# hangg7/soar

Hardware: AMD Instinct MI355X
Metric: fwd+bwd frames/sec @100k Gaussians, 1080p; achieved HBM GB/s vs roofline (higher is better)
Workload: dtype f32

## Files before the change

### include/soar_hip.h

```cpp
#ifndef SOAR_HIP_H
#define SOAR_HIP_H

#include <stddef.h>
#include <stdint.h>

#ifdef __cplusplus
extern "C" {
#endif

#define SOAR_HIP_ABI_VERSION 8

typedef struct SoarRastParams {
    int32_t P;
    int32_t W, H;
    int32_t sh_degree;
    int32_t M;
    int32_t prefiltered;
    int32_t render_front;
    int32_t sort_descending;
    int32_t debug;
    int32_t cfg_surface;
    int32_t cfg_normalize_depth;
    int32_t cfg_perpix_depth;
    int32_t cfg_lrn_cam;
// ... 108 lines not shown
int soar_lbs_knn_weights_bytes(int32_t P, int32_t V, size_t *bytes);
int soar_lbs_knn_weights(const float *xyz, int32_t P, const float *verts, int32_t V,
                         const float *vert_weights, int32_t J, int32_t K,
                         float *weights_out, int32_t *knn_idx_out,
                         void *workspace, size_t workspace_bytes, void *stream);

int soar_lbs_knn_grid_bytes(int32_t V, size_t *bytes);
int soar_lbs_knn_query_bytes(int32_t P, size_t *bytes);
int soar_lbs_knn_build_grid(const float *verts, int32_t V, const float *vert_weights, int32_t J, void *grid_buffer,
                            void *stream);
int soar_lbs_knn_query(const void *grid_buffer, int32_t V, const float *vert_weights, int32_t J,
                       const float *xyz, int32_t P, int32_t K, float *weights_out, int32_t *knn_idx_out,
                       void *query_workspace, size_t query_workspace_bytes, void *stream);
int soar_lbs_knn_query_ordered(const void *grid_buffer, int32_t V, const float *vert_weights, int32_t J,
                               const float *xyz, int32_t P, int32_t K, uint32_t *order, int32_t resort,
                               float *weights_out, int32_t *knn_idx_out,
                               void *query_workspace, size_t query_workspace_bytes, void *stream);

int soar_lbs_knn_state_bytes(int32_t P, size_t *bytes);
int soar_lbs_knn_query_state(const void *grid_buffer, int32_t V, const float *vert_weights, int32_t J, const float *xyz, int32_t P,
                             uint32_t *order, int32_t resort, float *weights_out, void *state_buffer, void *query_workspace,
                             size_t query_workspace_bytes, void *stream);
int soar_lbs_knn_refresh(const void *grid_buffer, int32_t V, int32_t J, const float *xyz, int32_t P, const uint32_t *order,
                         void *state_buffer, float *weights_out, uint32_t *searched_counter_dev, void *stream);

int soar_lbs_warp_forward(const float *xyz, const float *rot, const float *weights, const float *joint_mats,
                          const float *offsets, const float *axis_perm, int32_t P, int32_t J,
                          float *xyz_out, float *rot_out, float *pt_mats_out, void *stream);

int soar_lbs_warp_backward(const float *xyz, const float *rot, const float *weights, const float *joint_mats,
                           const float *axis_perm, int32_t P, int32_t J,
                           const float *dL_dxyz_out, const float *dL_drot_out,
                           float *dL_dxyz, float *dL_drot, void *stream);

typedef struct SoarFrameHead {
    const SoarRastParams *prm;
    void *geom_buffer;
    int32_t *radii;
} SoarFrameHead;
int soar_frames_warp_preprocess(int32_t n, const SoarFrameHead *frames, const float *xyz, const float *rot, const float *weights,
                                const float *joint_mats, int32_t P, int32_t J, const float *colors, const float *opacities, const float *scales,
                                float *xyz_out, float *rot_out, void *stream);

int soar_rast_backward_rows(const SoarRastParams *prm, const float *means3D, const int32_t *radii, const float *shs, const float *scales,
                            const float *rotations, const float *cov3D_precomp, const void *geom_buffer, const void *workspace,
                            float *dL_dmeans2D, float *dL_dcolors, float *dL_dopacity, float *dL_dmeans3D, float *dL_dcov3D, float *dL_dsh,
                            float *dL_dscales, float *dL_drotations, float *dL_dviewmat, float *dL_dprojmat, float *dL_dcampos, float *dL_docc,
                            void *stream);

typedef struct SoarFrameTail {
    const SoarRastParams *prm;
    const float *means3D;
    const float *rotations;
    const int32_t *radii;
    const void *geom_buffer;
    const void *workspace;
    float *dL_dmeans2D;
} SoarFrameTail;
int soar_frames_geometry_warp_backward(int32_t n, const SoarFrameTail *frames, const float *xyz, const float *rot, const float *weights,
                                       const float *joint_mats, int32_t P, int32_t J, const float *scales, float *dL_dxyz, float *dL_drot,
                                       float *dL_dscales, float *dL_dcolors, float *dL_docc, void *stream);

int soar_lbs_warp_forward_batch(const float *xyz, const float *rot, const float *weights, const float *joint_mats, int32_t n,
                                int32_t P, int32_t J, float *xyz_out, float *rot_out, void *stream);
int soar_lbs_warp_backward_sum(const float *xyz, const float *rot, const float *weights, const float *joint_mats, int32_t n,
                               int32_t P, int32_t J, const float *dL_dxyz_out, const float *dL_drot_out, float *dL_dxyz,
                               float *dL_drot, int32_t n_extra, const float *const *extra_src, float *const *extra_dst,
                               const int32_t *extra_width, void *stream);

int soar_dist2_knn3(const float *points, int32_t N, float *out, void *stream);

#define SOAR_FRAME_LOSS_SCRATCH_FLOATS (4 * 2048)
int soar_frame_loss(int32_t W, int32_t H, const float *color, const float *normal, const float *depth,
                    const float *opac, const float *target_color, const float *target_mask,
                    const float *target_normal, float w_color, float w_mask, float w_normal, float w_depth,
                    float *loss_out, float *scratch, float *dL_dcolor, float *dL_dnormal, float *dL_ddepth,
                    float *dL_dopac, const void *image_buffer, const float *background, int32_t normalize_depth, void *stream);

int soar_frame_loss_pooled(int32_t W, int32_t H, const float *color, const float *normal, const float *depth,
                           const float *opac, const float *target_pool, int32_t n_sets, const int32_t *set_index_dev,
                           float w_color, float w_mask, float w_normal, float w_depth, float *loss_out, float *scratch,
                           float *dL_dcolor, float *dL_dnormal, float *dL_ddepth, float *dL_dopac, const void *image_buffer,
                           const float *background, int32_t normalize_depth, void *stream);

typedef struct SoarAvatarLossArgs {
    int32_t H, W;
    float cos_limit, cos_weight;
    const float *render, *gt_rgb;
    const float *mask_img, *gt_mask;
    const float *normal, *gt_normal;
    const float *occ;
    const uint8_t *sel, *sel_normal, *sel_occ;
    float *stats, *stats_occ;
    float *scratch;
    const float *counts;
    const float *up_l1, *up_l1m, *up_cos, *up_occ, *up_ssim;
    const float *g_ssim;
    float *g_render, *g_mask, *g_normal, *g_occ;
    int32_t normal_raw;
    int32_t occ_grad_summed;
    float *cos_scale_out;
    const float *background;
} SoarAvatarLossArgs;
int soar_avatar_loss_scratch_floats(size_t *count);
int soar_avatar_pixel_losses(const SoarAvatarLossArgs *args, int32_t mode, void *stream);

int soar_ssim_scratch_floats(int32_t C, int32_t H, int32_t W, size_t *count);
int soar_ssim(int32_t C, int32_t H, int32_t W, const float *img1, const float *img2, float *ssim_out, float *scratch,
              float *dssim_dimg1, void *stream);
int soar_ssim_rendered(int32_t C, int32_t H, int32_t W, const float *img1, const float *img2, float *ssim_out, float *scratch,
                       float *dssim_dimg1, const float *rendered, void *stream);

typedef struct SoarDensifyRow {
    const float *src;
    float *dst;
    int32_t width;
    int32_t mode;
} SoarDensifyRow;
int soar_densify_stats(int32_t P, const int32_t *radii, const float *grad2d, int32_t grad_stride, const float *scaling_grad,
                       const float *rotation, const float *opacity, float *accum, float *max_radii2D, void *stream);
int soar_densify_plan_bytes(int32_t P, size_t *bytes);
int soar_densify_plan(int32_t P, const float *accum, const float *scaling, const float *opacity, int32_t do_prune,
                      int32_t do_densify, float min_opacity, float prune_scale_max, float prune_area_min, float max_grad,
                      float dense_scale, void *plan, int64_t *counts_host, void *stream);
int soar_densify_flags(int32_t P, const void *plan, uint8_t *flags_out, void *stream);
int soar_densify_apply(int32_t P, int32_t N, const void *plan, int32_t n_rows, const SoarDensifyRow *rows, const float *scaling,
                       const float *rotation, const float *noise, int32_t surface, void *stream);

int soar_smplx_joint_mats(int32_t B, int32_t J, int32_t NB, const float *betas, int32_t betas_batch, const float *J_template,
                          const float *J_dirs, const int32_t *parents, const float *full_pose, const float *transl,
                          const float *right_mats, float *out, void *stream);

int soar_image_loss_scratch_floats(size_t *count);
int soar_masked_l1(int32_t C, int32_t H, int32_t W, const float *img, const float *gt, const uint8_t *mask, float *stats2,
                   float *scratch, void *stream);
int soar_masked_l1_backward(int32_t C, int32_t H, int32_t W, const float *img, const float *gt, const uint8_t *mask,
                            const float *stats2, const float *upstream_dev, float *dL_dimg, void *stream);
int soar_cos_loss(int32_t C, int32_t H, int32_t W, const float *output, const float *gt, const uint8_t *mask, float cos_thrsh,
                  float weight, float *stats2, float *scratch, void *stream);
int soar_cos_loss_backward(int32_t C, int32_t H, int32_t W, const float *output, const float *gt, const uint8_t *mask,
                           float cos_thrsh, float weight, const float *stats2, const float *upstream_dev, float *dL_doutput,
                           void *stream);

int soar_depth2normal(int32_t W, int32_t H, const float *depth, const uint8_t *mask, float prcp_x, float prcp_y,
                      float focal_k00, float focal_k11, float *normal_out, void *stream);
int soar_depth2normal_backward(int32_t W, int32_t H, const float *depth, const uint8_t *mask, float prcp_x, float prcp_y,
                               float focal_k00, float focal_k11, const float *dL_dnormal, float *dL_ddepth, void *stream);
int soar_normal2curv(int32_t W, int32_t H, const float *normal, const uint8_t *mask, float *curv_out, void *stream);
int soar_normal2curv_backward(int32_t W, int32_t H, const float *normal, const uint8_t *mask, const float *dL_dcurv,
                              float *dL_dnormal, void *stream);

int soar_view_finish(int32_t W, int32_t H, const float *normal, const float *depth, const float *opac,
                     const float *prcppoint_dev, float focal_k00, float focal_k11, float *normal_out, float *curv_out,
                     float *pred_normal_out, void *stream);
int soar_view_finish_backward(int32_t W, int32_t H, const float *normal, const float *depth, const float *opac,
                              const float *prcppoint_dev, float focal_k00, float focal_k11, const float *dL_dnormal_out,
                              const float *dL_dcurv, const float *dL_dpred_normal, const float *dL_ddepth_direct,
                              float *dL_dnormal_and_depth, void *stream);

typedef struct SoarPoseArgs {
    int32_t P, J;
    int32_t scale_width;
    int32_t warp;
    const float *xyz, *rot;
    const float *weights;
    const float *joint_mats;
    const float *offsets;
    const float *axis_perm;
    const float *colors;
    const float *scale_src;
    const float *occ;
    float *occ3;
    float *posed;
    float *grad_scratch;
    float *dL_dxyz, *dL_drot, *dL_dcolors, *dL_dscale;
    float *dL_docc;
} SoarPoseArgs;
typedef struct SoarViewArgs {
    SoarRastParams rast;
    float focal_k00, focal_k11;
    int32_t back;
    int32_t pad_;
    int64_t capacity;
    void *buffer;
    size_t buffer_bytes;
    float *out;
    int32_t *radii;
    uint32_t *status_pinned;
    const float *g_render, *g_normal, *g_depth, *g_pred_normal, *g_mask, *g_occ, *g_curv;
    float *dL_dmeans2D;
} SoarViewArgs;
int soar_view_buffer_bytes(int32_t P, int32_t W, int32_t H, int64_t capacity, int32_t back, size_t *bytes);
int soar_views_grad_scratch_floats(int32_t P, int32_t n_views, size_t *floats);
int soar_views_forward(const SoarPoseArgs *pose, int32_t n_views, const SoarViewArgs *views, void *stream);
int soar_views_backward(const SoarPoseArgs *pose, int32_t n_views, const SoarViewArgs *views, void *stream);
int soar_step_views_forward(int32_t n_poses, const SoarPoseArgs *poses, const int32_t *views_per_pose, const SoarViewArgs *views, void *stream);
int soar_step_views_backward(int32_t n_poses, const SoarPoseArgs *poses, const int32_t *views_per_pose, const SoarViewArgs *views, void *stream);
typedef struct SoarCameraSpec {
    double fovx, fovy, znear, zfar;
    double cx, cy, img_w, img_h;
    int32_t has_cxcy, pad_;
} SoarCameraSpec;
int soar_cameras_from_c2w(int32_t n, const float *c2w_dev, const float *c2w_host, const SoarCameraSpec *specs, float *out_dev, void *stream);
int soar_rast_forward_render_status(const SoarRastParams *prm, const int32_t *radii, void *geom_buffer, void *binning_buffer,
                                    void *image_buffer, int64_t num_rendered, float *out_color, float *out_normal, float *out_depth,
                                    float *out_opac, const float *occ_values, float *out_occ, uint32_t *status_pinned, void *stream);
int soar_lbs_warp_backward_views(const float *xyz, const float *rot, const float *weights, const float *joint_mats, const float *axis_perm,
                                 int32_t n, int32_t P, int32_t J, const float *dL_dxyz_out, const float *dL_drot_out, float *dL_dxyz,
                                 float *dL_drot, int32_t n_extra, const float *const *extra_src, float *const *extra_dst,
                                 const int32_t *extra_width, void *stream);

int soar_prof_enable(int on);
int soar_prof_reset(void);
int soar_prof_stage_count(void);
const char *soar_prof_stage_name(int stage);
int soar_prof_read(int stage, double *total_ms, int64_t *launches);
int soar_sum_frames(int32_t n_frames, int64_t count, const float *in_dev, float *out_dev, void *stream);
int soar_gather_step_inputs(int32_t n_frames, int32_t num_frames_seq, int32_t floats_per_frame, int32_t n_sets,
                            const int32_t *frame_ids_dev, const float *table_dev, float *mats_out_dev,
                            int32_t *set_index_out_dev, void *stream);
int soar_gather_step_inputs_ids(int32_t n_frames, int32_t num_frames_seq, int32_t floats_per_frame, int32_t n_sets,
                                const int32_t *frame_ids_host, const float *table_dev, float *mats_out_dev,
                                int32_t *set_index_out_dev, void *stream);

typedef struct SoarAdamRow {
    float *param;
    const float *grad;
    float *exp_avg;
    float *exp_avg_sq;
    int64_t count;
    float lr;
    int32_t pad_;
} SoarAdamRow;
int soar_adam_step(int32_t n_rows, const SoarAdamRow *rows_host, double beta1, double beta2, double eps, void *state_dev, void *stream);
int soar_adam_step_at(int32_t n_rows, const SoarAdamRow *rows, double beta1, double beta2, double eps, int64_t step, void *stream);
int soar_adam_step_rows(int32_t n_rows, const SoarAdamRow *rows, double beta1, double beta2, double eps, void *state_dev, int32_t advance,
                        void *stream);
int soar_adam_step_rows_wide(int32_t n_rows, const SoarAdamRow *rows, double beta1, double beta2, double eps, void *state_dev,
                             int32_t advance, void *stream);

int soar_prof_timestamp(unsigned long long *ring_dev, int64_t capacity, int64_t tag, void *stream);

int soar_selftest_affine_scan(const float *m64_dev, const float *b64_dev, float *out192_dev, void *stream);

int soar_selftest_exp(const float *x_dev, int32_t n, float *out_dev, float *expf_dev, void *stream);

int soar_tsdf_integrate(int32_t n_views, int32_t H, int32_t W, const float *depth, const float *opac, const float *viewmatrix,
                        const float *projmatrix, const float *prcppoint, float origin_x, float origin_y, float origin_z, float voxel,
                        int32_t X, int32_t Y, int32_t Z, float trunc, float znear, float min_opacity, float *sum, float *weight,
                        void *stream);
int soar_mc_workspace_bytes(int32_t X, int32_t Y, int32_t Z, size_t *bytes);
int soar_mc_count(int32_t X, int32_t Y, int32_t Z, const float *values, const uint8_t *valid, float level, void *workspace,
                  size_t workspace_bytes, int64_t *counts_host, void *stream);
int soar_mc_emit(int32_t X, int32_t Y, int32_t Z, const float *values, const uint8_t *valid, float level, const void *workspace,
                 size_t workspace_bytes, float *verts, int32_t *faces, void *stream);
int soar_mesh_filter_bytes(int32_t V, int32_t F, size_t *bytes);
int soar_mesh_filter_components(int32_t V, int32_t F, const float *verts, const int32_t *faces, int32_t min_faces, float min_diag_frac,
                                void *workspace, size_t workspace_bytes, float *verts_out, int32_t *faces_out, int64_t *counts_host,
                                void *stream);

#define SOAR_FIELD_LEVELS 16
#define SOAR_FIELD_HIDDEN 64
#define SOAR_FIELD_HEAD_FLOATS(in, out) (SOAR_FIELD_HIDDEN * (in) + SOAR_FIELD_HIDDEN + (out) * SOAR_FIELD_HIDDEN + (out))
typedef struct SoarFieldHead {
    const float *w1, *b1, *w2, *b2;
} SoarFieldHead;

typedef struct SoarFieldArgs {
    int32_t N;
    int32_t log2_T;
    int32_t normalized;
    int32_t pad_;
    float res[SOAR_FIELD_LEVELS];
    const float *xyz;
    const float *aabb;
    const float *table, *qtable;
    const float *z;
    SoarFieldHead head[5];
    float *enc, *qenc;
    float *out[5];
    const float *g_out[5];
    float *d_table, *d_qtable;
    float *d_head[5];
    float *d_xyz, *d_z;
} SoarFieldArgs;

int soar_field_workspace_bytes(int32_t N, size_t *bytes);
int soar_field_forward(const SoarFieldArgs *args, void *stream);
int soar_field_backward(const SoarFieldArgs *args, void *workspace, size_t workspace_bytes, void *stream);

#define SOAR_ENVMAP_ENC 9
#define SOAR_ENVMAP_HIDDEN 16
#define SOAR_ENVMAP_WEIGHTS (SOAR_ENVMAP_HIDDEN * SOAR_ENVMAP_ENC + SOAR_ENVMAP_HIDDEN * SOAR_ENVMAP_HIDDEN + 3 * SOAR_ENVMAP_HIDDEN)
typedef struct SoarEnvmapArgs {
    int32_t B, H, W;
    int32_t n_comp;
    int32_t color_rows;
    int32_t pad_;
    int64_t render_stride, mask_stride;
    int64_t g_comp_stride[4];
    const float *dirs;
    const float *w1, *w2, *w3;
    const float *color;
    const float *render, *mask;
    float *bg;
    float *comp;
// ... 138 lines not shown
```

### soar_amd/csrc/api.hip

```cpp
#include "soar_common.h"

#include <mutex>

#include <dlfcn.h>

#include <cstdarg>
#include <cstdio>
#include <cstring>

namespace soar {

static thread_local char g_error[1024] = "";

void set_error(const char *fmt, ...)
{
    va_list ap;
    va_start(ap, fmt);
    vsnprintf(g_error, sizeof(g_error), fmt, ap);
    va_end(ap);
}

int check_hip(hipError_t e, const char *what, const char *file, int line)
{
    if (e == hipSuccess) return 0;
    set_error("HIP error %d (%s) in %s at %s:%d", (int)e, hipGetErrorString(e), what, file, line);
    return 1;
}

int post_launch(const char *what, hipStream_t stream, int debug)
{
    hipError_t e = hipGetLastError();
    if (e == hipSuccess && (debug & 1)) e = hipStreamSynchronize(stream);
    if (e == hipSuccess) return 0;
    set_error("stage '%s' failed: HIP error %d (%s)", what, (int)e, hipGetErrorString(e));
    return 1;
}

BatchCtx &batch_ctx()
{
    static thread_local BatchCtx ctx;
    return ctx;
}

namespace {
constexpr int ZERO_RANGES = 5;
struct ZeroArgs { uint32_t *ptr[ZERO_RANGES]; size_t words[ZERO_RANGES]; size_t first_block[ZERO_RANGES + 1]; };
constexpr int ZERO_UNROLL = 8;
constexpr size_t ZERO_BLOCK_WORDS = 256 * 4 * ZERO_UNROLL;
__global__ void __launch_bounds__(256) zero_ranges_kernel(Batch<ZeroArgs> b)
{
    const ZeroArgs &z = b.v[blockIdx.y];
    if (blockIdx.x >= z.first_block[ZERO_RANGES]) return;
    int r = 0;
    while (r < ZERO_RANGES - 1 && blockIdx.x >= z.first_block[r + 1]) r++;
    const size_t b0 = ((size_t)blockIdx.x - z.first_block[r]) * ZERO_BLOCK_WORDS;
    uint32_t *p = z.ptr[r];
    const size_t n = z.words[r];
    if (b0 + ZERO_BLOCK_WORDS <= n && (reinterpret_cast<uintptr_t>(p) & 15) == 0) {
#pragma unroll
        for (int u = 0; u < ZERO_UNROLL; u++)
            *reinterpret_cast<uint4 *>(p + b0 + (size_t)u * 1024 + threadIdx.x * 4) = make_uint4(0u, 0u, 0u, 0u);
    } else {
        for (size_t w = b0 + threadIdx.x; w < n && w < b0 + ZERO_BLOCK_WORDS; w += 256) p[w] = 0u;
    }
}
}

int launch_zero_ranges(const ZeroRange *ranges, int count, hipStream_t stream)
{
    ZeroArgs z;
    size_t blocks = 0;
    if (count > ZERO_RANGES) { set_error("launch_zero_ranges: at most %d ranges", ZERO_RANGES); return 1; }
    for (int r = 0; r < ZERO_RANGES; r++) {
        z.first_block[r] = blocks;
        z.ptr[r] = r < count ? static_cast<uint32_t *>(ranges[r].ptr) : nullptr;
        z.words[r] = r < count ? ranges[r].bytes / 4 : 0;
        blocks += (z.words[r] + ZERO_BLOCK_WORDS - 1) / ZERO_BLOCK_WORDS;
    }
    z.first_block[ZERO_RANGES] = blocks;
    if (blocks == 0) return 0;
    SOAR_LAUNCH_BATCHED(zero_ranges_kernel, dim3((unsigned)blocks), dim3(256), 0, stream, z);
    return post_launch("zero_ranges", stream, 0);
}

namespace {
struct ProfSlot { hipEvent_t a, b; int stage; bool open; };
constexpr int PROF_SLOTS = 16384;
std::mutex g_prof_mutex;
bool g_prof_on = false;
ProfSlot g_slots[PROF_SLOTS];
int g_slot_used = 0;
bool g_slots_init = false;
double g_stage_ms[ST_COUNT];
long long g_stage_n[ST_COUNT];
const char *g_stage_names[ST_COUNT] = {"preprocess", "scan", "tile_lists", "depth_order", "tile_ranges", "render_forward",
                                       "render_backward", "geometry_backward", "lbs_knn_weights", "lbs_warp_forward",
                                       "lbs_warp_backward", "dist2_knn3", "frame_loss", "postops", "block_masks", "optimizer"};
void prof_drain()
{
    for (int i = 0; i < g_slot_used; i++) {
        float ms = 0.f;
        if (hipEventSynchronize(g_slots[i].b) == hipSuccess && hipEventElapsedTime(&ms, g_slots[i].a, g_slots[i].b) == hipSuccess) {
            g_stage_ms[g_slots[i].stage] += ms;
            g_stage_n[g_slots[i].stage] += 1;
        }
    }
    g_slot_used = 0;
}
}

namespace {
struct Roctx {
    int (*push)(const char *) = nullptr;
    int (*pop)() = nullptr;
    Roctx()
    {
        const char *on = getenv("SOAR_ROCTX");
        if (!on || on[0] == '0') return;
        void *h = dlopen("librocprofiler-sdk-roctx.so", RTLD_NOW | RTLD_GLOBAL);
        if (!h) h = dlopen("libroctx64.so", RTLD_NOW | RTLD_GLOBAL);
        if (!h) return;
        push = reinterpret_cast<int (*)(const char *)>(dlsym(h, "roctxRangePushA"));
        pop = reinterpret_cast<int (*)()>(dlsym(h, "roctxRangePop"));
        if (!push || !pop) push = nullptr;
    }
};
const Roctx &roctx()
{
    static const Roctx r;
    return r;
}
}

StageTimer::StageTimer(int stage, hipStream_t s) : slot(-1), stream(s)
{
    marked = roctx().push != nullptr;
    if (marked) (void)roctx().push(g_stage_names[stage]);
    if (!g_prof_on) return;
    if (batch_ctx().n && batch_ctx().f != batch_ctx().n - 1) return;
    {
        std::lock_guard<std::mutex> lock(g_prof_mutex);
        if (!g_slots_init) {
            for (int i = 0; i < PROF_SLOTS; i++) { (void)hipEventCreate(&g_slots[i].a); (void)hipEventCreate(&g_slots[i].b); }
            g_slots_init = true;
        }
        if (g_slot_used == PROF_SLOTS) return;
        slot = g_slot_used++;
        g_slots[slot].stage = stage;
    }
    (void)hipEventRecord(g_slots[slot].a, stream);
}
StageTimer::~StageTimer()
{
    if (slot >= 0) (void)hipEventRecord(g_slots[slot].b, stream);
    if (marked) (void)roctx().pop();
}

template <typename T>
static void take(char *&p, T *&ptr, size_t count)
{
    p = reinterpret_cast<char *>(align_up(reinterpret_cast<size_t>(p)));
    ptr = reinterpret_cast<T *>(p);
// ... 446 lines not shown
                                     binning_buffer, image_buffer, num_rendered, dL_dout_color, dL_dout_normal, dL_dout_depth,
                                     dL_dout_opac, nullptr, dL_dmeans2D, dL_dcolors, dL_dopacity, dL_dmeans3D, dL_dcov3D, dL_dsh,
                                     dL_dscales, dL_drotations, dL_dviewmat, dL_dprojmat, dL_dcampos, workspace, workspace_bytes,
                                     stream_);
}

int soar_rast_backward_rows(const SoarRastParams *prm, const float *means3D, const int32_t *radii, const float *shs, const float *scales,
                            const float *rotations, const float *cov3D_precomp, const void *geom_buffer, const void *workspace,
                            float *dL_dmeans2D, float *dL_dcolors, float *dL_dopacity, float *dL_dmeans3D, float *dL_dcov3D, float *dL_dsh,
                            float *dL_dscales, float *dL_drotations, float *dL_dviewmat, float *dL_dprojmat, float *dL_dcampos, float *dL_docc,
                            void *stream_)
{
    hipStream_t stream = static_cast<hipStream_t>(stream_);
    if (check_params(prm)) return 1;
    if (prm->P == 0) return 0;
    if (check_aligned(geom_buffer, "geom_buffer") || check_aligned(workspace, "workspace")) return 1;
    if (!means3D || !radii || !dL_dmeans2D || !dL_dcolors || !dL_dopacity || !dL_dmeans3D || !dL_dcov3D || !dL_dscales || !dL_drotations ||
        !dL_dviewmat || !dL_dprojmat || !dL_dcampos) {
        set_error("soar_rast_backward_rows: a required pointer is NULL");
        return 1;
    }
    GeomBuf g;
    carve_geom(const_cast<void *>(geom_buffer), prm->P, prm->M, &g);
    return launch_geometry_backward(*prm, means3D, radii, shs, scales, rotations, cov3D_precomp, g, static_cast<const float *>(workspace),
                                    dL_dmeans2D, dL_dcolors, dL_dopacity, dL_dmeans3D, dL_dcov3D, dL_dsh, dL_dscales, dL_drotations,
                                    dL_dviewmat, dL_dprojmat, dL_dcampos, true, stream, dL_docc);
}

}

static int backward_impl(const SoarRastParams *prm, const float *means3D, const int32_t *radii, const float *shs,
                              const float *colors_precomp, const float *scales, const float *rotations,
                              const float *cov3D_precomp, const void *geom_buffer, const void *binning_buffer,
                              const void *image_buffer, int64_t num_rendered, const float *dL_dout_color,
                              const float *dL_dout_normal, const float *dL_dout_depth, const float *dL_dout_opac,
                              const float *grad_scale_dev, float *dL_dmeans2D, float *dL_dcolors, float *dL_dopacity,
                              float *dL_dmeans3D, float *dL_dcov3D, float *dL_dsh, float *dL_dscales, float *dL_drotations,
                              float *dL_dviewmat, float *dL_dprojmat, float *dL_dcampos, void *workspace,
                              size_t workspace_bytes, const float *dL_dout_occ, float *dL_docc, const float *normal_scale_dev, int occ_planes,
                              void *stream_)
{
    hipStream_t stream = static_cast<hipStream_t>(stream_);
    if (check_params(prm)) return 1;
    if (!dL_dviewmat || !dL_dprojmat || !dL_dcampos) { set_error("camera gradient pointers must not be NULL"); return 1; }
    if ((dL_dout_occ == nullptr) != (dL_docc == nullptr)) { set_error("soar_rast_backward_occ: dL_dout_occ and dL_docc go together"); return 1; }
    if (dL_dout_occ && (prm->render_front != 0 || prm->sort_descending != 0)) {
        set_error("soar_rast_backward_occ: the fused occlusion chain belongs to a main pass (render_front = 0, ascending)");
        return 1;
    }
    if (prm->P == 0) {
        SOAR_HIP_OK(hipMemsetAsync(dL_dviewmat, 0, 16 * sizeof(float), stream));
        SOAR_HIP_OK(hipMemsetAsync(dL_dprojmat, 0, 16 * sizeof(float), stream));
        SOAR_HIP_OK(hipMemsetAsync(dL_dcampos, 0, 3 * sizeof(float), stream));
        return 0;
    }
    if (check_aligned(geom_buffer, "geom_buffer") || check_aligned(image_buffer, "image_buffer") ||
        check_aligned(workspace, "workspace"))
        return 1;
    if (num_rendered > 0 && check_aligned(binning_buffer, "binning_buffer")) return 1;
    size_t need = 0;
    soar_rast_backward_workspace_bytes(prm->P, &need);
    if (workspace_bytes < need - ALIGN) { set_error("workspace too small: %zu < %zu", workspace_bytes, need); return 1; }
    if (!means3D || !radii || !dL_dout_color || !dL_dout_normal || !dL_dout_depth || !dL_dout_opac || !dL_dmeans2D ||
        !dL_dcolors || !dL_dopacity || !dL_dmeans3D || !dL_dcov3D || !dL_dscales || !dL_drotations) {
        set_error("soar_rast_backward: a required pointer is NULL");
        return 1;
    }
    if (prm->M > 0 && shs && !dL_dsh) { set_error("dL_dsh is NULL but SHs are in use"); return 1; }
    (void)colors_precomp;

    GeomBuf g;
    ImageBuf img;
    BinBuf b;
    carve_geom(const_cast<void *>(geom_buffer), prm->P, prm->M, &g);
    carve_image(const_cast<void *>(image_buffer), prm->W, prm->H, &img);
    carve_binning(const_cast<void *>(binning_buffer), num_rendered, &b);
    float *acc = static_cast<float *>(workspace);
    const bool wide = (prm->debug & 2) != 0;
    double *acc64 = wide ? reinterpret_cast<double *>(static_cast<char *>(workspace) + align_up(sizeof(float) * ACC_STRIDE * (size_t)prm->P))
                         : nullptr;
    {
        const ZeroRange zr[4] = {{wide ? (void *)acc64 : (void *)acc, (wide ? sizeof(double) : sizeof(float)) * ACC_STRIDE * (size_t)prm->P},
                                 {dL_dviewmat, 16 * sizeof(float)}, {dL_dprojmat, 16 * sizeof(float)}, {dL_dcampos, 3 * sizeof(float)}};
        if (launch_zero_ranges(zr, 4, stream)) return 1;
    }
    if (num_rendered > 0 || wide) {
        if (launch_render_backward(*prm, g, b, img, dL_dout_color, dL_dout_normal, dL_dout_depth, dL_dout_opac, grad_scale_dev, acc,
                                   acc64, num_rendered > 0, dL_dout_occ, dL_docc, normal_scale_dev, occ_planes, stream))
            return 1;
    }
    if ((prm->debug & 8) != 0) return 0;
    if (launch_geometry_backward(*prm, means3D, radii, shs, scales, rotations, cov3D_precomp, g, acc, dL_dmeans2D, dL_dcolors,
                                 dL_dopacity, dL_dmeans3D, dL_dcov3D, dL_dsh, dL_dscales, dL_drotations, dL_dviewmat,
                                 dL_dprojmat, dL_dcampos, false, stream, dL_docc))
        return 1;
    return 0;
}


extern "C" {

int soar_rast_backward_scaled(const SoarRastParams *prm, const float *means3D, const int32_t *radii, const float *shs,
                              const float *colors_precomp, const float *scales, const float *rotations,
                              const float *cov3D_precomp, const void *geom_buffer, const void *binning_buffer,
                              const void *image_buffer, int64_t num_rendered, const float *dL_dout_color,
                              const float *dL_dout_normal, const float *dL_dout_depth, const float *dL_dout_opac,
                              const float *grad_scale_dev, float *dL_dmeans2D, float *dL_dcolors, float *dL_dopacity,
                              float *dL_dmeans3D, float *dL_dcov3D, float *dL_dsh, float *dL_dscales, float *dL_drotations,
                              float *dL_dviewmat, float *dL_dprojmat, float *dL_dcampos, void *workspace,
                              size_t workspace_bytes, void *stream_)
{
    return backward_impl(prm, means3D, radii, shs, colors_precomp, scales, rotations, cov3D_precomp, geom_buffer, binning_buffer, image_buffer,
                         num_rendered, dL_dout_color, dL_dout_normal, dL_dout_depth, dL_dout_opac, grad_scale_dev, dL_dmeans2D, dL_dcolors,
                         dL_dopacity, dL_dmeans3D, dL_dcov3D, dL_dsh, dL_dscales, dL_drotations, dL_dviewmat, dL_dprojmat, dL_dcampos, workspace,
                         workspace_bytes, nullptr, nullptr, nullptr, 3, stream_);
}

int soar_rast_backward_occ(const SoarRastParams *prm, const float *means3D, const int32_t *radii, const float *shs,
                           const float *colors_precomp, const float *scales, const float *rotations,
                           const float *cov3D_precomp, const void *geom_buffer, const void *binning_buffer,
                           const void *image_buffer, int64_t num_rendered, const float *dL_dout_color,
                           const float *dL_dout_normal, const float *dL_dout_depth, const float *dL_dout_opac,
                           const float *dL_dout_occ, const float *normal_scale_dev, int32_t occ_planes, float *dL_dmeans2D, float *dL_dcolors,
                           float *dL_dopacity,
                           float *dL_dmeans3D, float *dL_dcov3D, float *dL_dsh, float *dL_dscales, float *dL_drotations,
                           float *dL_dviewmat, float *dL_dprojmat, float *dL_dcampos, float *dL_docc, void *workspace,
                           size_t workspace_bytes, void *stream_)
{
    if (!dL_dout_occ || !dL_docc) { set_error("soar_rast_backward_occ: dL_dout_occ / dL_docc must not be NULL"); return 1; }
    if (occ_planes != 1 && occ_planes != 3) { set_error("soar_rast_backward_occ: occ_planes is 3 or 1, got %d", occ_planes); return 1; }
    return backward_impl(prm, means3D, radii, shs, colors_precomp, scales, rotations, cov3D_precomp, geom_buffer, binning_buffer, image_buffer,
                         num_rendered, dL_dout_color, dL_dout_normal, dL_dout_depth, dL_dout_opac, nullptr, dL_dmeans2D, dL_dcolors,
                         dL_dopacity, dL_dmeans3D, dL_dcov3D, dL_dsh, dL_dscales, dL_drotations, dL_dviewmat, dL_dprojmat, dL_dcampos, workspace,
                         workspace_bytes, dL_dout_occ, dL_docc, normal_scale_dev, occ_planes, stream_);
}

int soar_rast_mark_visible(int32_t P, const float *means3D, const float *viewmatrix, const float *projmatrix,
                           uint8_t *present, void *stream_)
{
    (void)means3D; (void)viewmatrix; (void)projmatrix;
    hipStream_t stream = static_cast<hipStream_t>(stream_);
    if (P < 0) { set_error("P < 0"); return 1; }
    if (P == 0) return 0;
    if (!present) { set_error("present is NULL"); return 1; }
    SOAR_HIP_OK(hipMemsetAsync(present, 0, (size_t)P, stream));
    return 0;
}

}

namespace soar {
namespace {
__global__ void export_records_kernel(int P, const GaussRec *rec, float *means2D, float *depths, float *conic_opacity,
                                      float *normal, float *depth_plane, float *rgb)
{
    const int i = blockIdx.x * blockDim.x + threadIdx.x;
    if (i >= P) return;
    const GaussRec r = rec[i];
    if (means2D) { means2D[2 * i] = r.q0.x; means2D[2 * i + 1] = r.q0.y; }
    if (depths) depths[i] = r.q1.z;
    if (conic_opacity) {
        conic_opacity[4 * i] = r.q0.z; conic_opacity[4 * i + 1] = r.q0.w; conic_opacity[4 * i + 2] = r.q1.x;
        conic_opacity[4 * i + 3] = r.q1.y;
    }
    if (normal) { normal[3 * i] = r.q3.x; normal[3 * i + 1] = r.q3.y; normal[3 * i + 2] = r.q3.z; }
    if (depth_plane) { depth_plane[2 * i] = r.q1.w; depth_plane[2 * i + 1] = r.q2.x; }
    if (rgb) { rgb[3 * i] = r.q2.y; rgb[3 * i + 1] = r.q2.z; rgb[3 * i + 2] = r.q2.w; }
// ... 105 lines not shown
```

### soar_amd/csrc/frame_loss.hip

```cpp
#include "soar_common.h"

#include <type_traits>

namespace soar {

namespace {

struct LossArgs {
    int n;
    const float *color, *normal, *depth, *opac;
    const float *t_color, *t_mask, *t_normal;
    float wc, wm, wn, wd;
    float *dcolor, *dnormal, *ddepth, *dopac;
    float *sums;
    const int *set_index;
    int n_sets;
    const float *bg;
    int normalize_depth;
    const uint32_t *n_contrib;
    const uint32_t *bg_tiles;
    int W, gx;
};

__device__ __forceinline__ float sign_of(float v) { return v > 0.f ? 1.f : (v < 0.f ? -1.f : 0.f); }

__device__ __forceinline__ float wave_sum(float v)
{
#pragma unroll
    for (int off = 32; off > 0; off >>= 1) v += __shfl_xor(v, off);
    return v;
}

template <int V> struct Vec;
template <> struct Vec<4> { typedef float4 type; };
template <> struct Vec<1> { typedef float type; };
__device__ __forceinline__ float4 ld(const float4 *p, int i) { return p[i]; }
__device__ __forceinline__ float4 ld(const float *p, int i) { return make_float4(p[i], 0.f, 0.f, 0.f); }
__device__ __forceinline__ void st(float4 *p, int i, float4 v) { p[i] = v; }
__device__ __forceinline__ void st(float *p, int i, float4 v) { p[i] = v.x; }
__device__ __forceinline__ bool any_contrib(const uint4 *p, int i) { const uint4 v = p[i]; return (v.x | v.y | v.z | v.w) != 0u; }
__device__ __forceinline__ bool any_contrib(const uint32_t *p, int i) { return p[i] != 0u; }

template <int V>
__global__ void __launch_bounds__(256) frame_loss_kernel(Batch<LossArgs> batch)
{
    LossArgs a = batch.v[blockIdx.y];
    typedef typename Vec<V>::type T;
    const int nv = a.n / V;
    if (a.set_index) {
        const float *set = a.t_color + (size_t)((unsigned)*a.set_index % (unsigned)a.n_sets) * 7u * (size_t)a.n;
        a.t_color = set; a.t_mask = set + 3 * (size_t)a.n; a.t_normal = set + 4 * (size_t)a.n;
    }
    float s_c = 0.f, s_m = 0.f, s_n = 0.f, s_d = 0.f;
    const float gc = a.wc / (3.f * a.n), gm = a.wm / a.n, gn = a.wn / (3.f * a.n), gd = a.wd / a.n;
    const float4 pad = V == 4 ? make_float4(1.f, 1.f, 1.f, 1.f) : make_float4(1.f, 0.f, 0.f, 0.f);
    typedef typename std::conditional<V == 4, uint4, uint32_t>::type U;
    const float Tc = (float)(1 - 0.000001);
    const bool known = a.n_contrib && a.bg;
    float bgc[3] = {0.f, 0.f, 0.f};
    if (known) { bgc[0] = 0.f + Tc * a.bg[0]; bgc[1] = 0.f + Tc * a.bg[1]; bgc[2] = 0.f + Tc * a.bg[2]; }
    const float bg_depth = a.normalize_depth ? 0.f / (1.f - Tc) : 0.f + Tc * 10.f, bg_opac = 1.f - Tc;
    for (int i = blockIdx.x * 256 + threadIdx.x; i < nv; i += gridDim.x * 256) {
        bool wr = true;
        if (a.n_contrib) {
            bool empty_tile = false;
            if (a.bg_tiles) {
                const int p = i * V, y = p / a.W, x = p - y * a.W;
                empty_tile = a.bg_tiles[(y >> 4) * a.gx + (x >> 4)] != 0u;
            }
            wr = !empty_tile && any_contrib(reinterpret_cast<const U *>(a.n_contrib), i);
        }
        const bool rd = wr || !known;
        float4 nsum = make_float4(0.f, 0.f, 0.f, 0.f);
#pragma unroll
        for (int ch = 0; ch < 3; ch++) {
            const float4 c = rd ? ld(reinterpret_cast<const T *>(a.color + (size_t)ch * a.n), i) : make_float4(bgc[ch], bgc[ch], bgc[ch], bgc[ch]);
            const float4 t = ld(reinterpret_cast<const T *>(a.t_color + (size_t)ch * a.n), i);
            const float4 d = make_float4(c.x - t.x, c.y - t.y, c.z - t.z, c.w - t.w);
            s_c += (fabsf(d.x) + fabsf(d.y)) + (fabsf(d.z) + fabsf(d.w));
            if (wr) st(reinterpret_cast<T *>(a.dcolor + (size_t)ch * a.n), i,
                       make_float4(gc * sign_of(d.x), gc * sign_of(d.y), gc * sign_of(d.z), gc * sign_of(d.w)));
            const float4 nr = rd ? ld(reinterpret_cast<const T *>(a.normal + (size_t)ch * a.n), i) : make_float4(0.f, 0.f, 0.f, 0.f);
            const float4 nt = rd ? ld(reinterpret_cast<const T *>(a.t_normal + (size_t)ch * a.n), i) : make_float4(0.f, 0.f, 0.f, 0.f);
            nsum.x += nr.x * nt.x; nsum.y += nr.y * nt.y; nsum.z += nr.z * nt.z; nsum.w += nr.w * nt.w;
            if (wr) st(reinterpret_cast<T *>(a.dnormal + (size_t)ch * a.n), i, make_float4(gn * nt.x, gn * nt.y, gn * nt.z, gn * nt.w));
        }
        s_n += (nsum.x + nsum.y) + (nsum.z + nsum.w);
        const float4 o = rd ? ld(reinterpret_cast<const T *>(a.opac), i) : make_float4(bg_opac, bg_opac, bg_opac, bg_opac);
        const float4 m = ld(reinterpret_cast<const T *>(a.t_mask), i);
        const float4 e = make_float4(o.x - m.x, o.y - m.y, o.z - m.z, o.w - m.w);
        s_m += (fabsf(e.x) + fabsf(e.y)) + (fabsf(e.z) + fabsf(e.w));
        if (wr) st(reinterpret_cast<T *>(a.dopac), i, make_float4(gm * sign_of(e.x), gm * sign_of(e.y), gm * sign_of(e.z), gm * sign_of(e.w)));
        const float4 dp = rd ? ld(reinterpret_cast<const T *>(a.depth), i) : make_float4(bg_depth, bg_depth, bg_depth, bg_depth);
        s_d += (dp.x + dp.y) + (dp.z + dp.w);
        if (wr) st(reinterpret_cast<T *>(a.ddepth), i, make_float4(gd * pad.x, gd * pad.y, gd * pad.z, gd * pad.w));
    }
    __shared__ float part[4][4];
    s_c = wave_sum(s_c); s_m = wave_sum(s_m); s_n = wave_sum(s_n); s_d = wave_sum(s_d);
    const int wave = threadIdx.x >> 6, lane = threadIdx.x & 63;
    if (lane == 0) { part[wave][0] = s_c; part[wave][1] = s_m; part[wave][2] = s_n; part[wave][3] = s_d; }
    __syncthreads();
    if (threadIdx.x < 4)
        a.sums[4 * blockIdx.x + threadIdx.x] = (part[0][threadIdx.x] + part[1][threadIdx.x]) + (part[2][threadIdx.x] + part[3][threadIdx.x]);
}

struct LossFinishArgs {
    const float *sums;
    int blocks, n;
    float wc, wm, wn, wd;
    float *loss;
};
__global__ void __launch_bounds__(256) frame_loss_finish_kernel(Batch<LossFinishArgs> batch)
{
    const LossFinishArgs &fa = batch.v[blockIdx.y];
    const float *sums = fa.sums;
    const int blocks = fa.blocks, n = fa.n;
    const float wc = fa.wc, wm = fa.wm, wn = fa.wn, wd = fa.wd;
    float *loss = fa.loss;
    __shared__ float4 red[256];
    float4 acc = make_float4(0.f, 0.f, 0.f, 0.f);
    for (int b = threadIdx.x; b < blocks; b += 256) {
        const float4 v = reinterpret_cast<const float4 *>(sums)[b];
        acc.x += v.x; acc.y += v.y; acc.z += v.z; acc.w += v.w;
    }
    red[threadIdx.x] = acc;
    __syncthreads();
    for (int off = 128; off > 0; off >>= 1) {
        if ((int)threadIdx.x < off) {
            const float4 o = red[threadIdx.x + off];
            float4 m = red[threadIdx.x];
            m.x += o.x; m.y += o.y; m.z += o.z; m.w += o.w;
            red[threadIdx.x] = m;
        }
        __syncthreads();
    }
    if (threadIdx.x == 0) {
        const float4 S = red[0];
        *loss = (wc * S.x / (3.f * n) + wm * S.y / n) + (wn * S.z / (3.f * n) + wd * S.w / n);
    }
}

}

}

using namespace soar;

static int frame_loss_launch(int32_t W, int32_t H, const float *color, const float *normal, const float *depth, const float *opac,
                             const float *target_color, const float *target_mask, const float *target_normal,
                             const int32_t *set_index_dev, int32_t n_sets, float w_color, float w_mask, float w_normal,
                             float w_depth, float *loss_out, float *sums4, float *dL_dcolor, float *dL_dnormal, float *dL_ddepth,
                             float *dL_dopac, const void *image_buffer, const float *background, int32_t normalize_depth, hipStream_t stream);

extern "C" int soar_frame_loss(int32_t W, int32_t H, const float *color, const float *normal, const float *depth,
                               const float *opac, const float *target_color, const float *target_mask,
                               const float *target_normal, float w_color, float w_mask, float w_normal, float w_depth,
                               float *loss_out, float *sums4, float *dL_dcolor, float *dL_dnormal, float *dL_ddepth,
                               float *dL_dopac, const void *image_buffer, const float *background, int32_t normalize_depth,
                               void *stream_)
{
    return frame_loss_launch(W, H, color, normal, depth, opac, target_color, target_mask, target_normal, nullptr, 1, w_color,
                             w_mask, w_normal, w_depth, loss_out, sums4, dL_dcolor, dL_dnormal, dL_ddepth, dL_dopac, image_buffer,
                             background, normalize_depth, static_cast<hipStream_t>(stream_));
}

extern "C" int soar_frame_loss_pooled(int32_t W, int32_t H, const float *color, const float *normal, const float *depth,
                                      const float *opac, const float *target_pool, int32_t n_sets,
                                      const int32_t *set_index_dev, float w_color, float w_mask, float w_normal, float w_depth,
                                      float *loss_out, float *sums4, float *dL_dcolor, float *dL_dnormal, float *dL_ddepth,
                                      float *dL_dopac, const void *image_buffer, const float *background,
                                      int32_t normalize_depth, void *stream_)
{
    if (n_sets <= 0 || !set_index_dev) { set_error("soar_frame_loss_pooled: need n_sets > 0 and a device index"); return 1; }
    return frame_loss_launch(W, H, color, normal, depth, opac, target_pool, target_pool, target_pool, set_index_dev, n_sets,
                             w_color, w_mask, w_normal, w_depth, loss_out, sums4, dL_dcolor, dL_dnormal, dL_ddepth, dL_dopac,
                             image_buffer, background, normalize_depth, static_cast<hipStream_t>(stream_));
}

static int frame_loss_launch(int32_t W, int32_t H, const float *color, const float *normal, const float *depth, const float *opac,
                             const float *target_color, const float *target_mask, const float *target_normal,
                             const int32_t *set_index_dev, int32_t n_sets, float w_color, float w_mask, float w_normal,
                             float w_depth, float *loss_out, float *sums4, float *dL_dcolor, float *dL_dnormal, float *dL_ddepth,
                             float *dL_dopac, const void *image_buffer, const float *background, int32_t normalize_depth, hipStream_t stream)
{
    if (W <= 0 || H <= 0) { set_error("soar_frame_loss: bad image size %dx%d", W, H); return 1; }
    if (!color || !normal || !depth || !opac || !target_color || !target_mask || !target_normal || !loss_out || !sums4 ||
        !dL_dcolor || !dL_dnormal || !dL_ddepth || !dL_dopac) {
        set_error("soar_frame_loss: NULL pointer");
        return 1;
    }
    LossArgs a;
    a.n = W * H;
    a.color = color; a.normal = normal; a.depth = depth; a.opac = opac;
    a.t_color = target_color; a.t_mask = target_mask; a.t_normal = target_normal;
    a.wc = w_color; a.wm = w_mask; a.wn = w_normal; a.wd = w_depth;
    a.dcolor = dL_dcolor; a.dnormal = dL_dnormal; a.ddepth = dL_ddepth; a.dopac = dL_dopac;
    a.sums = sums4;
    a.set_index = set_index_dev; a.n_sets = n_sets;
    a.n_contrib = nullptr; a.bg_tiles = nullptr; a.W = W; a.gx = (W + TILE - 1) / TILE;
    a.bg = image_buffer ? background : nullptr; a.normalize_depth = normalize_depth;
    if (image_buffer) {
        ImageBuf img;
        carve_image(const_cast<void *>(image_buffer), W, H, &img);
        a.n_contrib = img.n_contrib;
        if (W % 4 == 0) a.bg_tiles = img.bg_tiles;
    }
    StageTimer timer(ST_FRAME_LOSS, stream);
    const bool vec4 = (a.n & 3) == 0 && (((uintptr_t)a.n_contrib | (uintptr_t)color | (uintptr_t)normal | (uintptr_t)depth | (uintptr_t)opac | (uintptr_t)target_color |
                                          (uintptr_t)target_mask | (uintptr_t)target_normal | (uintptr_t)dL_dcolor | (uintptr_t)dL_dnormal |
                                          (uintptr_t)dL_ddepth | (uintptr_t)dL_dopac) & 15) == 0;
    const int blocks = min(SOAR_FRAME_LOSS_SCRATCH_FLOATS / 4, max(1, (a.n / (vec4 ? 4 : 1) + 255) / 256));
    if (vec4) SOAR_LAUNCH_BATCHED(frame_loss_kernel<4>, dim3(blocks), dim3(256), 0, stream, a);
    else SOAR_LAUNCH_BATCHED(frame_loss_kernel<1>, dim3(blocks), dim3(256), 0, stream, a);
    const soar::LossFinishArgs fa = {sums4, blocks, a.n, w_color, w_mask, w_normal, w_depth, loss_out};
    SOAR_LAUNCH_BATCHED(frame_loss_finish_kernel, dim3(1), dim3(256), 0, stream, fa);
    SOAR_LAUNCH_OK("frame_loss", stream, 0);
    return 0;
}


namespace soar {
namespace {
template <int VEC>
__global__ void __launch_bounds__(256) sum_frames_kernel(int n_frames, size_t count, const float *__restrict__ in, float *__restrict__ out)
{
    const size_t i = ((size_t)blockIdx.x * 256 + threadIdx.x) * VEC;
    if (i >= count) return;
    if (VEC == 4) {
        float4 acc = *reinterpret_cast<const float4 *>(in + i);
        for (int f = 1; f < n_frames; f++) {
            const float4 v = *reinterpret_cast<const float4 *>(in + (size_t)f * count + i);
            acc.x += v.x; acc.y += v.y; acc.z += v.z; acc.w += v.w;
        }
        *reinterpret_cast<float4 *>(out + i) = acc;
    } else {
        float acc = in[i];
        for (int f = 1; f < n_frames; f++) acc += in[(size_t)f * count + i];
        out[i] = acc;
    }
}
__global__ void gather_step_inputs_kernel(int n_frames, int num_frames_seq, int floats_per_frame, int n_sets,
                                          const int32_t *__restrict__ frame_ids, const float *__restrict__ table,
                                          float *__restrict__ mats_out, int32_t *__restrict__ set_out)
{
    const int f = blockIdx.x;
    int id = frame_ids[f] % num_frames_seq;
    if (id < 0) id += num_frames_seq;
    for (int k = threadIdx.x; k < floats_per_frame; k += blockDim.x) mats_out[(size_t)f * floats_per_frame + k] = table[(size_t)id * floats_per_frame + k];
    if (threadIdx.x == 0 && set_out) set_out[f] = n_sets > 0 ? id % n_sets : 0;
}
struct StepFrameIds { int32_t id[MAX_BATCH]; };
__global__ void gather_step_inputs_ids_kernel(int n_frames, int num_frames_seq, int floats_per_frame, int n_sets, StepFrameIds ids,
                                              const float *__restrict__ table, float *__restrict__ mats_out, int32_t *__restrict__ set_out)
{
    const int f = blockIdx.x;
    int id = ids.id[f] % num_frames_seq;
    if (id < 0) id += num_frames_seq;
    for (int k = threadIdx.x; k < floats_per_frame; k += blockDim.x) mats_out[(size_t)f * floats_per_frame + k] = table[(size_t)id * floats_per_frame + k];
    if (threadIdx.x == 0 && set_out) set_out[f] = n_sets > 0 ? id % n_sets : 0;
}
}
}

extern "C" int soar_sum_frames(int32_t n_frames, int64_t count, const float *in_dev, float *out_dev, void *stream_)
{
    using namespace soar;
    hipStream_t stream = static_cast<hipStream_t>(stream_);
    if (n_frames <= 0 || count < 0 || !in_dev || !out_dev) { set_error("soar_sum_frames: bad arguments"); return 1; }
    if (count == 0) return 0;
    const bool vec = ((((uintptr_t)in_dev | (uintptr_t)out_dev) & 15) == 0) && ((count & 3) == 0);
    if (vec) hipLaunchKernelGGL(sum_frames_kernel<4>, dim3((unsigned)((count / 4 + 255) / 256)), dim3(256), 0, stream, n_frames, (size_t)count, in_dev, out_dev);
    else hipLaunchKernelGGL(sum_frames_kernel<1>, dim3((unsigned)((count + 255) / 256)), dim3(256), 0, stream, n_frames, (size_t)count, in_dev, out_dev);
    SOAR_LAUNCH_OK("sum_frames", stream, 0);
    return 0;
}

extern "C" int soar_gather_step_inputs(int32_t n_frames, int32_t num_frames_seq, int32_t floats_per_frame, int32_t n_sets,
                                       const int32_t *frame_ids_dev, const float *table_dev, float *mats_out_dev,
                                       int32_t *set_index_out_dev, void *stream_)
{
    using namespace soar;
    hipStream_t stream = static_cast<hipStream_t>(stream_);
    if (n_frames <= 0 || num_frames_seq <= 0 || floats_per_frame <= 0 || !frame_ids_dev || !table_dev || !mats_out_dev) {
        set_error("soar_gather_step_inputs: bad arguments");
        return 1;
    }
    hipLaunchKernelGGL(gather_step_inputs_kernel, dim3(n_frames), dim3(256), 0, stream, n_frames, num_frames_seq, floats_per_frame, n_sets,
                       frame_ids_dev, table_dev, mats_out_dev, set_index_out_dev);
    SOAR_LAUNCH_OK("gather_step_inputs", stream, 0);
    return 0;
}

extern "C" int soar_gather_step_inputs_ids(int32_t n_frames, int32_t num_frames_seq, int32_t floats_per_frame, int32_t n_sets,
                                           const int32_t *frame_ids_host, const float *table_dev, float *mats_out_dev,
                                           int32_t *set_index_out_dev, void *stream_)
{
    using namespace soar;
    hipStream_t stream = static_cast<hipStream_t>(stream_);
    if (n_frames <= 0 || n_frames > MAX_BATCH || num_frames_seq <= 0 || floats_per_frame <= 0 || !frame_ids_host || !table_dev || !mats_out_dev) {
        set_error("soar_gather_step_inputs_ids: bad arguments (at most %d frames per step)", MAX_BATCH);
        return 1;
    }
    StepFrameIds ids = {};
    for (int f = 0; f < n_frames; f++) ids.id[f] = frame_ids_host[f];
    hipLaunchKernelGGL(gather_step_inputs_ids_kernel, dim3(n_frames), dim3(256), 0, stream, n_frames, num_frames_seq, floats_per_frame, n_sets, ids,
                       table_dev, mats_out_dev, set_index_out_dev);
    SOAR_LAUNCH_OK("gather_step_inputs", stream, 0);
    return 0;
}
```

### soar_amd/csrc/lbs_knn.hip

```cpp
#include "soar_common.h"

#include <cstdio>
#include <cstdlib>
#include <cstring>
#include <rocprim/device/device_radix_sort.hpp>

namespace soar {

namespace {

constexpr int KNN_THREADS = 128;
constexpr int KNN_MAXK = 32;
constexpr int GRID_MAX = 64;
constexpr int GRID_RES = 28;
constexpr int KNN_K = 30;
constexpr int KNN_JMAX = 56;
constexpr int GRID_CELLS = GRID_MAX * GRID_MAX * GRID_MAX;

struct GridMeta {
    float minx, miny, minz, h, inv_h;
    int nx, ny, nz;
};

__global__ void __launch_bounds__(256) grid_meta_kernel(const float *__restrict__ verts, int V, GridMeta *meta)
// ... 336 lines not shown
    for (int k = 0; k < K; k++) {
        v[k] = fminf(best[k], other[(K - 1 - k) * stride]);
        tau = fmaxf(tau, v[k]);
    }
    need = K;
#pragma unroll
    for (int k = 0; k < K; k++) need -= (v[k] < tau) ? 1 : 0;
    return tau;
}

constexpr uint32_t KNN_ORDER_STAMP = 0x534F4152u;
__global__ void __launch_bounds__(WAVE)
item_cost_kernel(const uint32_t *__restrict__ q_keys, int P, const GridMeta *__restrict__ meta, const uint2 *__restrict__ cell_range,
                 uint32_t *__restrict__ cost)
{
    const int lane = threadIdx.x, chunk = blockIdx.x, q = chunk * WAVE + lane;
    const bool valid = q < P;
    const uint32_t key = valid ? q_keys[q] : 0xFFFFFFFFu;
    const GridMeta m = *meta;
    uint32_t item[KNN_SLOTS];
#pragma unroll
    for (int k = 0; k < KNN_SLOTS; k++) item[k] = 0u;
    unsigned long long remaining = __ballot(valid);
    for (int seg = 0; remaining != 0ull; seg++) {
        const uint32_t c = (uint32_t)__builtin_amdgcn_readlane((int)key, (int)__builtin_ctzll(remaining));
        const unsigned long long mine = __ballot(valid && key == c);
        remaining &= ~mine;
        const int cx = (int)(c % GRID_MAX), cy = (int)((c / GRID_MAX) % GRID_MAX), cz = (int)(c / (GRID_MAX * GRID_MAX));
        uint32_t n = 0;
        if (lane < 27) {
            const int gx = cx + lane % 3 - 1, gy = cy + (lane / 3) % 3 - 1, gz = cz + lane / 9 - 1;
            if (gx >= 0 && gx < m.nx && gy >= 0 && gy < m.ny && gz >= 0 && gz < m.nz) {
                const uint2 rg = cell_range[(gz * GRID_MAX + gy) * GRID_MAX + gx];
                n = rg.y - rg.x;
            }
        }
#pragma unroll
        for (int off = 16; off > 0; off >>= 1) n += (uint32_t)__shfl_xor((int)n, off);
        n = (uint32_t)__builtin_amdgcn_readfirstlane((int)n);
        if (n < 2u * KNN_K) {
            uint32_t n5 = 0;
            for (int t = lane; t < 125; t += WAVE) {
                const int gx = cx + t % 5 - 2, gy = cy + (t / 5) % 5 - 2, gz = cz + t / 25 - 2;
                if (gx >= 0 && gx < m.nx && gy >= 0 && gy < m.ny && gz >= 0 && gz < m.nz) {
                    const uint2 rg = cell_range[(gz * GRID_MAX + gy) * GRID_MAX + gx];
                    n5 += rg.y - rg.x;
                }
            }
#pragma unroll
            for (int off = 32; off > 0; off >>= 1) n5 += (uint32_t)__shfl_xor((int)n5, off);
            n += (uint32_t)__builtin_amdgcn_readfirstlane((int)n5);
        }
        const uint32_t us100 = 8u * n + 70u * (uint32_t)__builtin_popcountll(mine) + 1200u;
#pragma unroll
        for (int k = 0; k < KNN_SLOTS; k++) item[k] += (seg % KNN_SLOTS) == k ? us100 : 0u;
    }
    if (lane < KNN_SLOTS) cost[chunk * KNN_SLOTS + lane] = lane == 0 ? item[0] : lane == 1 ? item[1] : lane == 2 ? item[2] : item[3];
}
__global__ void __launch_bounds__(1024) item_order_kernel(const uint32_t *__restrict__ cost, int n_items, uint32_t *__restrict__ order)
{
    __shared__ uint32_t count[33], cursor[33];
    const int tid = threadIdx.x;
    if (tid < 33) count[tid] = 0u;
    __syncthreads();
    auto class_of = [&](uint32_t c) -> int { return c == 0u ? 32 : 31 - (int)min(31u, c / 400u); };
    for (int i = tid; i < n_items; i += 1024) atomicAdd(&count[class_of(cost[i])], 1u);
    __syncthreads();
    if (tid == 0) {
        uint32_t acc = 0;
        for (int k = 0; k < 33; k++) { cursor[k] = acc; acc += count[k]; }
    }
    __syncthreads();
    for (int i = tid; i < n_items; i += 1024) order[atomicAdd(&cursor[class_of(cost[i])], 1u)] = (uint32_t)i;
    if (tid == 0) order[n_items] = KNN_ORDER_STAMP ^ (uint32_t)n_items;
}

template <bool WITH_IDX>
__global__ void __launch_bounds__(KNN_WAVES *WAVE) __attribute__((amdgpu_waves_per_eu(5, 8)))
knn_cell_kernel(const float *__restrict__ xyz, int P, int V, const GridMeta *__restrict__ meta,
                const uint2 *__restrict__ cell_range, const float4 *__restrict__ sorted_verts,
                const uint32_t *__restrict__ q_keys, const uint32_t *__restrict__ q_ids,
                const float *__restrict__ rows_padded, int J, float *__restrict__ weights_out,
                int32_t *__restrict__ knn_idx_out, const uint32_t *__restrict__ item_order,
                KnnStatePtrs state)
{
    constexpr int K = KNN_K;
    __shared__ float4 cand[KNN_CAND];
    __shared__ uint32_t row_start[KNN_ROWS], row_prefix[KNN_ROWS + 1];
    __shared__ int info[4];
    __shared__ float merge[2][K][WAVE];
    __shared__ float tau_s[WAVE];
    __shared__ int need_s[WAVE];
    __shared__ uint32_t list_pos[KNN_WAVES][WAVE];
    __shared__ float list_w[KNN_WAVES][WAVE];

    const int wave = threadIdx.x >> 6, lane = threadIdx.x & 63;
    const uint32_t n_items = gridDim.x;
    const bool ordered = item_order && item_order[n_items] == (KNN_ORDER_STAMP ^ n_items);
    const uint32_t n_chunks = n_items / KNN_SLOTS;
    const uint32_t item = ordered ? min(item_order[blockIdx.x], n_items - 1u) : (blockIdx.x % n_chunks) * KNN_SLOTS + blockIdx.x / n_chunks;
    const int chunk = (int)(item / KNN_SLOTS), slot = (int)(item % KNN_SLOTS);
    const int q = chunk * WAVE + lane;
    const bool valid = q < P;
    const uint32_t key = valid ? q_keys[q] : 0xFFFFFFFFu;
    unsigned long long remaining = __ballot(valid);
    if (remaining == 0ull) return;

    const int p = valid ? (int)q_ids[q] : 0;
    const float x = xyz[3 * p], y = xyz[3 * p + 1], z = xyz[3 * p + 2];
    const GridMeta m = *meta;
    const float qx = x - m.minx, qy = y - m.miny, qz = z - m.minz;

    for (int seg = 0; remaining != 0ull; seg++) {
        const int head = (int)__builtin_ctzll(remaining);
        const uint32_t c = (uint32_t)__builtin_amdgcn_readlane((int)key, head);
        const bool active = valid && key == c;
        remaining &= ~__ballot(active);
        if ((seg % KNN_SLOTS) != slot) continue;
        const int cx = (int)(c % GRID_MAX), cy = (int)((c / GRID_MAX) % GRID_MAX), cz = (int)(c / (GRID_MAX * GRID_MAX));

        int r = 1, n_rows = 0, N = 0;
        for (;; r++) {
            __syncthreads();
            if (wave == 0) box_rows(cell_range, m, cx, cy, cz, r, V, row_start, row_prefix, info, lane);
            __syncthreads();
            N = info[0];
            n_rows = info[1];
            float best[K];
#pragma unroll
            for (int k = 0; k < K; k++) best[k] = 3.0e38f;
            for (int base = 0; base < N; base += KNN_CAND) {
                const int n = min(KNN_CAND, N - base);
                if (base > 0) __syncthreads();
                stage_candidates(sorted_verts, row_start, row_prefix, n_rows, base, n, cand);
                __syncthreads();
#pragma unroll 2
                for (int i = wave; i < n; i += KNN_WAVES) chain_insert<K>(best, dist2_exact(x, y, z, cand[i]));
            }
            if (wave >= 2) {
#pragma unroll
                for (int k = 0; k < K; k++) merge[wave - 2][k][lane] = best[k];
            }
            __syncthreads();
            if (wave < 2) merge_sorted<K>(best, &merge[wave][0][lane], WAVE);
            __syncthreads();
            if (wave == 1) {
#pragma unroll
                for (int k = 0; k < K; k++) merge[0][k][lane] = best[k];
            }
            __syncthreads();
            if (wave == 0) {
                int need;
                const float tau = merge_sorted_kth<K>(best, &merge[0][0][lane], WAVE, need);
                tau_s[lane] = tau;
                need_s[lane] = need;
                float bound = 3.0e38f;
                bool open = false;
                if (cx - r > 0) { open = true; bound = fminf(bound, qx - (cx - r) * m.h); }
                if (cx + r < m.nx - 1) { open = true; bound = fminf(bound, (cx + r + 1) * m.h - qx); }
                if (cy - r > 0) { open = true; bound = fminf(bound, qy - (cy - r) * m.h); }
                if (cy + r < m.ny - 1) { open = true; bound = fminf(bound, (cy + r + 1) * m.h - qy); }
                if (cz - r > 0) { open = true; bound = fminf(bound, qz - (cz - r) * m.h); }
                if (cz + r < m.nz - 1) { open = true; bound = fminf(bound, (cz + r + 1) * m.h - qz); }
                bound = fmaxf(bound, 0.f) * 0.9999f;
                const bool certified = !open || r > KNN_RMAX || tau <= bound * bound;
                const bool final_box = __ballot(active && !certified) == 0ull;
                if (lane == 0) info[2] = final_box ? 1 : 0;
            }
            __syncthreads();
            if (info[2]) break;
        }
        const float tau = tau_s[lane];
        const int need = need_s[lane];

        const bool single = N <= KNN_CAND;
        float norm_lane = 0.f;
        int cnt_lane = 0;
        int need_left = need;
        uint32_t *lpos = list_pos[wave];
        float *lw = list_w[wave];
// ... 117 lines not shown
constexpr int KNN_FSLOTS = 4;
struct KnnSlots { uint2 list[KNN_FSLOTS][KNN_KEEP]; int p[KNN_FSLOTS]; };
__device__ __forceinline__ void slots_fill_pair(KnnSlots &sl, int slot_lo, int p, uint32_t mask, uint32_t pos, float d2, int lane)
{
    const int slot = slot_lo + (lane >> 5), l5 = lane & (KNN_KEEP - 1);
    if (p >= 0 && ((mask >> l5) & 1u)) {
        const int at = __builtin_popcount(mask & ((1u << l5) - 1u));
        sl.list[slot][at] = make_uint2(pos * (uint32_t)(KNN_JMAX * sizeof(float)), __float_as_uint(1.0f / fminf(fmaxf(sqrtf(d2), 0.0001f), 1.0f)));
    }
    if (l5 == 0) sl.p[slot] = p;
}
template <int UNROLL>
__device__ __forceinline__ void slots_blend(KnnSlots &sl, int lane, const float *__restrict__ rows_padded, int J,
                                            float *__restrict__ weights_out)
{
    static_assert(KNN_K % 2 == 0 && KNN_JMAX % 4 == 0 && KNN_JMAX / 4 <= 16 && KNN_FSLOTS * 16 == WAVE && KNN_KEEP * 2 == WAVE &&
                  KNN_JMAX * sizeof(float) <= KNN_KEEP * sizeof(uint2) && KNN_JMAX <= WAVE, "slot layout");
    __builtin_amdgcn_fence(__ATOMIC_RELEASE, "wavefront");
    __builtin_amdgcn_wave_barrier();
    __builtin_amdgcn_fence(__ATOMIC_ACQUIRE, "wavefront");
    const int g = lane >> 4, t = lane & 15;
    const int p = sl.p[g];
    if (p >= 0) {
        const uint32_t t16 = (uint32_t)min(t, KNN_JMAX / 4 - 1) * 16u;
        const char *rows_bytes = reinterpret_cast<const char *>(rows_padded);
        const uint4 *mine = reinterpret_cast<const uint4 *>(sl.list[g]);
        float4 acc = make_float4(0.f, 0.f, 0.f, 0.f);
        float norm = 0.f;
#pragma unroll UNROLL
        for (int k2 = 0; k2 < KNN_K / 2; k2++) {
            const uint4 e = mine[k2];
            const float4 r0 = *reinterpret_cast<const float4 *>(rows_bytes + (e.x + t16));
            const float4 r1 = *reinterpret_cast<const float4 *>(rows_bytes + (e.z + t16));
            const float w0 = __uint_as_float(e.y), w1 = __uint_as_float(e.w);
            acc.x = __builtin_fmaf(w0, r0.x, acc.x); acc.y = __builtin_fmaf(w0, r0.y, acc.y);
            acc.z = __builtin_fmaf(w0, r0.z, acc.z); acc.w = __builtin_fmaf(w0, r0.w, acc.w);
            norm += w0;
            acc.x = __builtin_fmaf(w1, r1.x, acc.x); acc.y = __builtin_fmaf(w1, r1.y, acc.y);
            acc.z = __builtin_fmaf(w1, r1.z, acc.z); acc.w = __builtin_fmaf(w1, r1.w, acc.w);
            norm += w1;
        }
        float4 *mine_out = reinterpret_cast<float4 *>(sl.list[g]);
        if (t < KNN_JMAX / 4) mine_out[t] = make_float4(acc.x / norm, acc.y / norm, acc.z / norm, acc.w / norm);
    }
    __builtin_amdgcn_fence(__ATOMIC_RELEASE, "wavefront");
    __builtin_amdgcn_wave_barrier();
    __builtin_amdgcn_fence(__ATOMIC_ACQUIRE, "wavefront");
#pragma unroll
    for (int r = 0; r < KNN_FSLOTS; r++) {
        const int pr = sl.p[r];
        if (pr >= 0 && lane < J) weights_out[(size_t)pr * J + lane] = reinterpret_cast<const float *>(sl.list[r])[lane];
    }
    __builtin_amdgcn_fence(__ATOMIC_RELEASE, "wavefront");
    __builtin_amdgcn_wave_barrier();
}

__device__ __forceinline__ uint32_t rank_32_halves(float d2, int lane, float &h30)
{
    const int l5 = lane & (KNN_KEEP - 1), base = lane & KNN_KEEP;
    int rank = 0;
#pragma unroll
    for (int j = 0; j < KNN_KEEP; j++) {
        const float dj = __shfl(d2, base + j);
        rank += (dj < d2 || (dj == d2 && j < l5)) ? 1 : 0;
    }
    const bool in = rank < KNN_K;
    float d_in = in ? d2 : 0.f, d_out = in ? 3.0e38f : d2;
#pragma unroll
    for (int off = KNN_KEEP / 2; off > 0; off >>= 1) {
        d_in = fmaxf(d_in, __shfl_xor(d_in, off));
        d_out = fminf(d_out, __shfl_xor(d_out, off));
    }
    h30 = half_gap(d_in, d_out);
    const unsigned long long b = __ballot(in);
    return (uint32_t)(base ? (b >> 32) : b);
}

#ifndef SOAR_KNN_CERT_PAIRS
#define SOAR_KNN_CERT_PAIRS 2
#endif
constexpr int KNN_CERT_PAIRS = SOAR_KNN_CERT_PAIRS;
__global__ void __launch_bounds__(KNN_WAVES *WAVE)
knn_certify_kernel(const float *__restrict__ xyz, int P, const float4 *__restrict__ sorted_verts, const uint32_t *__restrict__ order,
                   KnnStatePtrs st)
{
    const int wave = threadIdx.x >> 6, lane = threadIdx.x & 63, l5 = lane & (KNN_KEEP - 1);
    const int q_base = ((int)blockIdx.x * KNN_WAVES + wave) * (2 * KNN_CERT_PAIRS) + (lane >> 5);
    if (q_base - (lane >> 5) >= P) return;
    int qs[KNN_CERT_PAIRS];
    float4 ra[KNN_CERT_PAIRS], rb[KNN_CERT_PAIRS], vv[KNN_CERT_PAIRS];
    float xs[KNN_CERT_PAIRS], ys[KNN_CERT_PAIRS], zs[KNN_CERT_PAIRS];
#pragma unroll
    for (int i = 0; i < KNN_CERT_PAIRS; i++) {
        qs[i] = q_base + 2 * i;
        const int qc = min(qs[i], P - 1);
        const int p = order ? (int)order[qc] : qc;
        const uint32_t pos = st.nbr[(size_t)qc * KNN_STATE_STRIDE + l5];
        ra[i] = st.ref30[qc]; rb[i] = st.ref32[qc];
        xs[i] = xyz[3 * p]; ys[i] = xyz[3 * p + 1]; zs[i] = xyz[3 * p + 2];
        vv[i] = sorted_verts[pos];
    }
#pragma unroll
    for (int i = 0; i < KNN_CERT_PAIRS; i++) {
        const int q = qs[i];
        const bool valid = q < P;
        const float x = xs[i], y = ys[i], z = zs[i];
        const float d2 = dist2_exact(x, y, z, vv[i]);
        const float ax = x - ra[i].x, ay = y - ra[i].y, az = z - ra[i].z, bx = x - rb[i].x, by = y - rb[i].y, bz = z - rb[i].z;
        const float moved_a = __builtin_amdgcn_sqrtf((ax * ax + ay * ay) + az * az) * 1.0001f + 1.0e-12f;
        const float moved_b = __builtin_amdgcn_sqrtf((bx * bx + by * by) + bz * bz) * 1.0001f + 1.0e-12f;
        const bool ok_a = ra[i].w > 0.f && moved_a < ra[i].w, ok_b = rb[i].w > 0.f && moved_b < rb[i].w;
        const bool tier3 = valid && !ok_a && !ok_b, tier2 = valid && !ok_a && ok_b;
        if (__ballot(tier3)) {
            float far = d2;
#pragma unroll
            for (int off = KNN_KEEP / 2; off > 0; off >>= 1) far = fmaxf(far, __shfl_xor(far, off));
            if (tier3 && l5 == 0) {
                const uint32_t list = knn_work_list_of((uint32_t)q);
                uint32_t *item = knn_work_item(st.work, P, list, atomicAdd(st.work + list * KNN_WORK_LINE, 1u));
                item[0] = (uint32_t)q;
                item[1] = __float_as_uint(far);
            }
        }
        if (__ballot(tier2)) {
            float h30;
            const uint32_t mask = rank_32_halves(d2, lane, h30);
            if (tier2 && l5 == 0) { st.ref30[q] = make_float4(x, y, z, h30); st.in30[q] = mask; }
        }
        if (valid) st.d2[(size_t)q * KNN_STATE_STRIDE + l5] = tier3 ? -1.f : d2;
    }
}

#ifndef SOAR_KNN_SEARCH_BLOCKS
#define SOAR_KNN_SEARCH_BLOCKS 768
#endif
#ifndef SOAR_KNN_BS_WPE
#define SOAR_KNN_BS_WPE 4
#endif
__global__ void __launch_bounds__(KNN_WAVES *WAVE) __attribute__((amdgpu_waves_per_eu(SOAR_KNN_BS_WPE, 8)))
knn_blend_search_kernel(const float *__restrict__ xyz, int P, int search_blocks, const GridMeta *__restrict__ meta,
                        const uint2 *__restrict__ cell_range, const float4 *__restrict__ sorted_verts, const float *__restrict__ rows_padded,
                        int J, const uint32_t *__restrict__ order, KnnStatePtrs st, float *__restrict__ weights_out,
                        uint32_t *__restrict__ counters)
{
    constexpr int KEEP = KNN_KEEP;
    __shared__ uint32_t c_pos[KNN_WAVES][RF_CAP];
    __shared__ float c_d[KNN_WAVES][RF_CAP];
    __shared__ uint32_t row_first[KNN_WAVES][WAVE], row_end[KNN_WAVES][WAVE];
    __shared__ __attribute__((aligned(16))) KnnSlots slots[KNN_WAVES];
    const int wave = threadIdx.x >> 6, lane = threadIdx.x & 63;
    if ((int)blockIdx.x >= search_blocks) {
        const int q0 = (((int)blockIdx.x - search_blocks) * KNN_WAVES + wave) * KNN_FSLOTS;
        if (q0 >= P) return;
        const int l5 = lane & (KNN_KEEP - 1);
        float dd[2];
        uint32_t pp[2], mm[2];
        int pq[2];
#pragma unroll
        for (int r = 0; r < 2; r++) {
            const int q = q0 + 2 * r + (lane >> 5);
            const size_t at = (size_t)min(q, P - 1) * KNN_STATE_STRIDE + l5;
            dd[r] = st.d2[at];
            pp[r] = st.nbr[at];
            mm[r] = st.in30[min(q, P - 1)];
            pq[r] = order ? (int)order[min(q, P - 1)] : min(q, P - 1);
            if (q >= P) dd[r] = -1.f;
        }
#pragma unroll
        for (int r = 0; r < 2; r++) slots_fill_pair(slots[wave], 2 * r, dd[r] >= 0.f ? pq[r] : -1, mm[r], pp[r], dd[r], lane);
        slots_blend<SOAR_KNN_SLOT_UNROLL>(slots[wave], lane, rows_padded, J, weights_out);
// ... 268 lines not shown
                           g.sorted_verts, g.rows);
    SOAR_LAUNCH_OK("lbs_knn_build_grid", stream, 0);
    return 0;
}

struct QueryWs {
    size_t sort_bytes, total;
    uint32_t *qk0, *qk1, *qv0, *qv1;
    uint32_t *item_cost, *item_order;
};
int carve_query_ws(void *base, int32_t P, QueryWs *out, hipStream_t stream)
{
    size_t qsort_bytes = 0;
    (void)rocprim::radix_sort_pairs((void *)nullptr, qsort_bytes, (uint32_t *)nullptr, (uint32_t *)nullptr,
                                    (uint32_t *)nullptr, (uint32_t *)nullptr, (size_t)(P > 0 ? P : 1), 0u, 18u, stream);
    size_t off = 0;
    auto carve = [&](size_t n) { size_t o = off; off = align_up(off + n); return o; };
    const size_t o_tmp = carve(qsort_bytes), o_qk0 = carve(4 * (size_t)P), o_qk1 = carve(4 * (size_t)P),
                 o_qv0 = carve(4 * (size_t)P), o_qv1 = carve(4 * (size_t)P), o_cost = carve(4 * KNN_SLOTS * (((size_t)P + WAVE - 1) / WAVE)),
                 o_ord = carve(4 * (KNN_SLOTS * (((size_t)P + WAVE - 1) / WAVE) + 1));
    (void)o_tmp;
    char *b = static_cast<char *>(base);
    out->sort_bytes = qsort_bytes;
    out->total = off;
    out->qk0 = reinterpret_cast<uint32_t *>(b + o_qk0); out->qk1 = reinterpret_cast<uint32_t *>(b + o_qk1);
    out->qv0 = reinterpret_cast<uint32_t *>(b + o_qv0); out->qv1 = reinterpret_cast<uint32_t *>(b + o_qv1);
    out->item_cost = reinterpret_cast<uint32_t *>(b + o_cost); out->item_order = reinterpret_cast<uint32_t *>(b + o_ord);
    return 0;
}

struct KnnState { KnnStatePtrs p; size_t total; };
int carve_knn_state(void *base, int32_t P, KnnState *out)
{
    char *b = static_cast<char *>(base);
    const size_t n = (size_t)(P > 0 ? P : 1);
    size_t off = 0;
    auto carve = [&](size_t bytes) { size_t o = off; off = align_up(off + bytes); return b + o; };
    out->p.nbr = reinterpret_cast<uint32_t *>(carve(sizeof(uint32_t) * KNN_STATE_STRIDE * n));
    out->p.ref30 = reinterpret_cast<float4 *>(carve(sizeof(float4) * n));
    out->p.ref32 = reinterpret_cast<float4 *>(carve(sizeof(float4) * n));
    out->p.in30 = reinterpret_cast<uint32_t *>(carve(sizeof(uint32_t) * n));
    out->p.work = reinterpret_cast<uint32_t *>(carve(sizeof(uint32_t) * knn_work_words(P)));
    out->p.d2 = reinterpret_cast<float *>(carve(sizeof(float) * KNN_STATE_STRIDE * n));
    out->total = off;
    return 0;
}

int knn_query(const KnnGrid &g, int32_t V, const float *vert_weights, int32_t J, const float *xyz, int32_t P, int32_t K,
              float *weights_out, int32_t *knn_idx_out, uint32_t *order, int resort, void *query_ws, size_t query_ws_bytes,
              hipStream_t stream, const KnnState *state = nullptr)
{
    const bool fast = (K == KNN_K) && (J <= KNN_JMAX);
    KnnStatePtrs st_none = {nullptr, nullptr, nullptr, nullptr, nullptr, nullptr};
    const KnnStatePtrs st = state ? state->p : st_none;
    if (!fast && state) { set_error("soar_lbs_knn: the neighbour state needs K = %d and J <= %d", KNN_K, KNN_JMAX); return 1; }
    if (!fast) {
        hipLaunchKernelGGL(knn_grid_kernel, dim3((P + KNN_THREADS - 1) / KNN_THREADS), dim3(KNN_THREADS), 0, stream, xyz, P, V,
                           g.meta, g.cell_range, g.sorted_verts, vert_weights, J, K, weights_out, knn_idx_out);
        SOAR_LAUNCH_OK("lbs_knn_weights", stream, 0);
        return 0;
    }
    QueryWs ws;
    if (carve_query_ws(query_ws, P, &ws, stream)) return 1;
    if (ws.total > query_ws_bytes) {
        set_error("soar_lbs_knn_query: query workspace too small (%zu bytes, need %zu for P=%d)", query_ws_bytes, ws.total, P);
        return 1;
    }
    size_t qsort_bytes = ws.sort_bytes;
    char *b = static_cast<char *>(query_ws);
    const size_t o_tmp = 0;
    uint32_t *qk0 = ws.qk0, *qk1 = ws.qk1, *qv0 = ws.qv0, *qv1 = ws.qv1;
    if (order && !resort) {
        hipLaunchKernelGGL(query_cells_ordered_kernel, dim3((P + 255) / 256), dim3(256), 0, stream, xyz, P, g.meta, order, qk1);
        qv1 = order;
    } else {
        hipLaunchKernelGGL(query_cells_kernel, dim3((P + 255) / 256), dim3(256), 0, stream, xyz, P, g.meta, qk0, qv0);
        SOAR_HIP_OK(rocprim::radix_sort_pairs(b + o_tmp, qsort_bytes, qk0, qk1, qv0, order ? order : qv1, (size_t)P, 0u, 18u,
                                              stream));
        if (order) qv1 = order;
        const int nchunks = (P + WAVE - 1) / WAVE;
        hipLaunchKernelGGL(item_cost_kernel, dim3(nchunks), dim3(WAVE), 0, stream, qk1, P, g.meta, g.cell_range, ws.item_cost);
        hipLaunchKernelGGL(item_order_kernel, dim3(1), dim3(1024), 0, stream, ws.item_cost, nchunks * KNN_SLOTS, ws.item_order);
    }
    const dim3 grid(((P + WAVE - 1) / WAVE) * KNN_SLOTS);
    if (knn_idx_out)
        hipLaunchKernelGGL(knn_cell_kernel<true>, grid, dim3(KNN_WAVES * WAVE), 0, stream, xyz, P, V, g.meta, g.cell_range,
                           g.sorted_verts, qk1, qv1, g.rows, J, weights_out, knn_idx_out, ws.item_order, st);
    else
        hipLaunchKernelGGL(knn_cell_kernel<false>, grid, dim3(KNN_WAVES * WAVE), 0, stream, xyz, P, V, g.meta, g.cell_range,
                           g.sorted_verts, qk1, qv1, g.rows, J, weights_out, knn_idx_out, ws.item_order, st);
    SOAR_LAUNCH_OK("lbs_knn_weights", stream, 0);
    return 0;
}

int check_knn_sizes(int32_t P, int32_t V, int32_t J, int32_t K)
{
    if (P < 0 || V <= 0 || J <= 0 || K <= 0) { set_error("soar_lbs_knn: bad sizes P=%d V=%d J=%d K=%d", P, V, J, K); return 1; }
    if (K > KNN_MAXK || K > V) { set_error("soar_lbs_knn: K=%d unsupported (max %d, V=%d)", K, KNN_MAXK, V); return 1; }
    return 0;
}

}

extern "C" int soar_lbs_knn_grid_bytes(int32_t V, size_t *bytes)
{
    if (V <= 0 || !bytes) { set_error("soar_lbs_knn_grid_bytes: bad arguments"); return 1; }
    KnnGrid g;
    if (carve_knn_grid(nullptr, V, &g, nullptr)) return 1;
    *bytes = g.total;
    return 0;
}

extern "C" int soar_lbs_knn_build_grid(const float *verts, int32_t V, const float *vert_weights, int32_t J, void *grid_buffer,
                                       void *stream_)
{
    hipStream_t stream = static_cast<hipStream_t>(stream_);
    if (V <= 0 || J <= 0 || !verts || !vert_weights || !grid_buffer) { set_error("soar_lbs_knn_build_grid: bad arguments"); return 1; }
    KnnGrid g;
    if (carve_knn_grid(grid_buffer, V, &g, stream)) return 1;
    return knn_build(verts, V, vert_weights, J, g, stream);
}

extern "C" int soar_lbs_knn_query_bytes(int32_t P, size_t *bytes)
{
    if (P < 0 || !bytes) { set_error("soar_lbs_knn_query_bytes: bad arguments"); return 1; }
    QueryWs ws;
    if (carve_query_ws(nullptr, P, &ws, nullptr)) return 1;
    *bytes = ws.total;
    return 0;
}

static int check_ws(const char *who, const void *ws, size_t have)
{
    if (!ws) { set_error("%s: NULL workspace (caller-owned, see the *_bytes query)", who); return 1; }
    if (reinterpret_cast<uintptr_t>(ws) % ALIGN) { set_error("%s: workspace is not %zu-byte aligned", who, ALIGN); return 1; }
    (void)have;
    return 0;
}

extern "C" int soar_lbs_knn_query(const void *grid_buffer, int32_t V, const float *vert_weights, int32_t J, const float *xyz,
                                  int32_t P, int32_t K, float *weights_out, int32_t *knn_idx_out, void *query_workspace,
                                  size_t query_workspace_bytes, void *stream_)
{
    hipStream_t stream = static_cast<hipStream_t>(stream_);
    if (check_knn_sizes(P, V, J, K)) return 1;
    if (P == 0) return 0;
    if (!grid_buffer || !xyz || !vert_weights || !weights_out) { set_error("soar_lbs_knn_query: NULL pointer"); return 1; }
    if (check_ws("soar_lbs_knn_query", query_workspace, query_workspace_bytes)) return 1;
    KnnGrid g;
    if (carve_knn_grid(const_cast<void *>(grid_buffer), V, &g, stream)) return 1;
    StageTimer timer(ST_LBS_KNN, stream);
    return knn_query(g, V, vert_weights, J, xyz, P, K, weights_out, knn_idx_out, nullptr, 1, query_workspace, query_workspace_bytes,
                     stream);
}

extern "C" int soar_lbs_knn_query_ordered(const void *grid_buffer, int32_t V, const float *vert_weights, int32_t J, const float *xyz,
                                          int32_t P, int32_t K, uint32_t *order, int32_t resort, float *weights_out,
                                          int32_t *knn_idx_out, void *query_workspace, size_t query_workspace_bytes, void *stream_)
{
    hipStream_t stream = static_cast<hipStream_t>(stream_);
    if (check_knn_sizes(P, V, J, K)) return 1;
    if (P == 0) return 0;
    if (!grid_buffer || !xyz || !vert_weights || !weights_out || !order) { set_error("soar_lbs_knn_query_ordered: NULL pointer"); return 1; }
    if (check_ws("soar_lbs_knn_query_ordered", query_workspace, query_workspace_bytes)) return 1;
    KnnGrid g;
    if (carve_knn_grid(const_cast<void *>(grid_buffer), V, &g, stream)) return 1;
    StageTimer timer(ST_LBS_KNN, stream);
    return knn_query(g, V, vert_weights, J, xyz, P, K, weights_out, knn_idx_out, order, resort, query_workspace,
                     query_workspace_bytes, stream);
}

extern "C" int soar_lbs_knn_state_bytes(int32_t P, size_t *bytes)
{
    if (P < 0 || !bytes) { set_error("soar_lbs_knn_state_bytes: bad arguments"); return 1; }
    KnnState st;
    carve_knn_state(nullptr, P, &st);
    *bytes = st.total;
    return 0;
}

extern "C" int soar_lbs_knn_query_state(const void *grid_buffer, int32_t V, const float *vert_weights, int32_t J, const float *xyz,
                                        int32_t P, uint32_t *order, int32_t resort, float *weights_out, void *state_buffer,
                                        void *query_workspace, size_t query_workspace_bytes, void *stream_)
{
    hipStream_t stream = static_cast<hipStream_t>(stream_);
    if (check_knn_sizes(P, V, J, KNN_K)) return 1;
    if (V < KNN_STATE_STRIDE) { set_error("soar_lbs_knn_query_state: the neighbour state keeps %d vertices per query, V=%d", KNN_STATE_STRIDE, V); return 1; }
    if (P == 0) return 0;
    if (!grid_buffer || !xyz || !vert_weights || !weights_out || !order || !state_buffer) { set_error("soar_lbs_knn_query_state: NULL pointer"); return 1; }
    if (check_ws("soar_lbs_knn_query_state", query_workspace, query_workspace_bytes) || check_ws("soar_lbs_knn_query_state", state_buffer, 0)) return 1;
    KnnGrid g;
    if (carve_knn_grid(const_cast<void *>(grid_buffer), V, &g, stream)) return 1;
    if (V <= KNN_KEEP) { set_error("soar_lbs_knn_query_state: the neighbour state keeps %d vertices per query, V = %d", KNN_KEEP, V); return 1; }
    KnnState st;
    carve_knn_state(state_buffer, P, &st);
    StageTimer timer(ST_LBS_KNN, stream);
    SOAR_HIP_OK(hipMemsetAsync(st.p.work, 0, KNN_WORK_LISTS * KNN_WORK_LINE * sizeof(uint32_t), stream));
    return knn_query(g, V, vert_weights, J, xyz, P, KNN_K, weights_out, nullptr, order, resort, query_workspace, query_workspace_bytes,
                     stream, &st);
}

extern "C" int soar_lbs_knn_refresh(const void *grid_buffer, int32_t V, int32_t J, const float *xyz, int32_t P, const uint32_t *order,
                                    void *state_buffer, float *weights_out, uint32_t *searched_counter_dev, void *stream_)
{
    hipStream_t stream = static_cast<hipStream_t>(stream_);
    if (check_knn_sizes(P, V, J, KNN_K)) return 1;
    if (J > KNN_JMAX) { set_error("soar_lbs_knn_refresh: J <= %d", KNN_JMAX); return 1; }
    if (V < KNN_STATE_STRIDE) { set_error("soar_lbs_knn_refresh: the neighbour state keeps %d vertices per query, V=%d", KNN_STATE_STRIDE, V); return 1; }
    if (P == 0) return 0;
    if (!grid_buffer || !xyz || !weights_out || !state_buffer || !order) { set_error("soar_lbs_knn_refresh: NULL pointer"); return 1; }
    if (check_ws("soar_lbs_knn_refresh", state_buffer, 0)) return 1;
    KnnGrid g;
    if (carve_knn_grid(const_cast<void *>(grid_buffer), V, &g, stream)) return 1;
    KnnState st;
    carve_knn_state(state_buffer, P, &st);
    StageTimer timer(ST_LBS_KNN, stream);
    const int per_block = KNN_WAVES * 2 * KNN_CERT_PAIRS, nblocks = (P + per_block - 1) / per_block;
    static_assert(SOAR_KNN_SEARCH_BLOCKS * KNN_WAVES % KNN_WORK_LISTS == 0, "searchers per list");
    hipLaunchKernelGGL(knn_certify_kernel, dim3(nblocks), dim3(KNN_WAVES * WAVE), 0, stream, xyz, P, g.sorted_verts, order, st.p);
    const int search_blocks = SOAR_KNN_SEARCH_BLOCKS, blend_blocks = (P + KNN_WAVES * KNN_FSLOTS - 1) / (KNN_WAVES * KNN_FSLOTS);
    hipLaunchKernelGGL(knn_blend_search_kernel, dim3(search_blocks + blend_blocks), dim3(KNN_WAVES * WAVE), 0, stream, xyz, P, search_blocks,
                       g.meta, g.cell_range, g.sorted_verts, g.rows, J, order, st.p, weights_out, searched_counter_dev);
    SOAR_LAUNCH_OK("lbs_knn_refresh", stream, 0);
    return 0;
}

extern "C" int soar_lbs_knn_weights_bytes(int32_t P, int32_t V, size_t *bytes)
{
    if (P < 0 || V <= 0 || !bytes) { set_error("soar_lbs_knn_weights_bytes: bad arguments"); return 1; }
    KnnGrid g;
    if (carve_knn_grid(nullptr, V, &g, nullptr)) return 1;
    QueryWs ws;
    if (carve_query_ws(nullptr, P, &ws, nullptr)) return 1;
    *bytes = align_up(g.total) + ws.total;
    return 0;
}

extern "C" int soar_lbs_knn_weights(const float *xyz, int32_t P, const float *verts, int32_t V, const float *vert_weights,
                                    int32_t J, int32_t K, float *weights_out, int32_t *knn_idx_out, void *workspace,
                                    size_t workspace_bytes, void *stream_)
{
    hipStream_t stream = static_cast<hipStream_t>(stream_);
    if (check_knn_sizes(P, V, J, K)) return 1;
    if (P == 0) return 0;
    if (!xyz || !verts || !vert_weights || !weights_out) { set_error("soar_lbs_knn_weights: NULL pointer"); return 1; }
    if (check_ws("soar_lbs_knn_weights", workspace, workspace_bytes)) return 1;
    KnnGrid g;
    if (carve_knn_grid(workspace, V, &g, stream)) return 1;
    QueryWs ws;
    if (carve_query_ws(nullptr, P, &ws, stream)) return 1;
    const size_t grid_part = align_up(g.total);
    if (workspace_bytes < grid_part + ws.total) {
        set_error("soar_lbs_knn_weights: workspace too small (%zu bytes, need %zu)", workspace_bytes, grid_part + ws.total);
        return 1;
    }
    StageTimer timer(ST_LBS_KNN, stream);
    if (knn_build(verts, V, vert_weights, J, g, stream)) return 1;
    return knn_query(g, V, vert_weights, J, xyz, P, K, weights_out, knn_idx_out, nullptr, 1,
                     static_cast<char *>(workspace) + grid_part, workspace_bytes - grid_part, stream);
}
```

### soar_amd/csrc/soar_common.h

```cpp
#pragma once

#include <hip/hip_runtime.h>
#include <cstdlib>
#include <type_traits>
#include <stdint.h>
#include <stddef.h>

#include "../../include/soar_hip.h"

namespace soar {

constexpr int TILE = 16;
constexpr int TILE_PIX = TILE * TILE;
constexpr int WAVE = 64;
constexpr size_t ALIGN = 256;

void set_error(const char *fmt, ...);
int check_hip(hipError_t e, const char *what, const char *file, int line);
#define SOAR_HIP_OK(expr)                                                         \
    do {                                                                          \
        if (::soar::check_hip((expr), #expr, __FILE__, __LINE__)) return 1;       \
    } while (0)
int post_launch(const char *what, hipStream_t stream, int debug);
#define SOAR_LAUNCH_OK(what, stream, debug)                                       \
// ... 221 lines not shown
__device__ __forceinline__ float mul_one_minus(float T, float alpha)
{
#pragma clang fp contract(off)
    return T * (1.f - alpha);
}
#endif

#if defined(__HIPCC__)
__device__ __forceinline__ uint32_t class_slot(uint32_t *counter, int cls, bool ok)
{
    const unsigned long long act = __ballot(ok);
    if (act == 0ull) return 0u;
    const int c0 = __builtin_amdgcn_readlane(cls, (int)__builtin_ctzll(act));
    const unsigned long long same = __ballot(ok && cls == c0);
    const int rank = (int)__builtin_amdgcn_mbcnt_hi((uint32_t)(same >> 32), __builtin_amdgcn_mbcnt_lo((uint32_t)same, 0u));
    uint32_t base = 0u;
    if (ok && cls == c0 && rank == 0) base = atomicAdd(&counter[c0], (uint32_t)__builtin_popcountll(same));
    base = (uint32_t)__builtin_amdgcn_readlane((int)base, (int)__builtin_ctzll(same));
    if (ok && cls != c0) return atomicAdd(&counter[cls], 1u);
    return base + (uint32_t)rank;
}

static __device__ __forceinline__ void tile_order_block(int T, int Tpad, const uint32_t *tile_count, const uint2 *ranges, uint32_t *order,
                                                        uint4 *order_rec, const float *bg, int normalize_depth, uint32_t *bg_state,
                                                        uint2 *empty_ranges = nullptr)
{
    __shared__ uint32_t count[16], cursor[16];
    const int tid = threadIdx.x, NTH = (int)blockDim.x;
    auto len_of = [&](int t) -> uint32_t { return empty_ranges ? 0u : tile_count ? tile_count[t] : ranges[t].y - ranges[t].x; };
    if (tid < 16) count[tid] = 0u;
    __syncthreads();
    if (empty_ranges)
        for (int t = tid; t < T; t += NTH) empty_ranges[t] = make_uint2(0u, 0u);
    for (int t0 = 0; t0 < T; t0 += 8 * NTH) {
        uint32_t len[8];
#pragma unroll
        for (int k = 0; k < 8; k++) {
            const int t = t0 + k * NTH + tid;
            len[k] = t < T ? len_of(t) : 0u;
        }
#pragma unroll
        for (int k = 0; k < 8; k++) {
            const int cls = 15 - min(15, 32 - __clz((int)len[k]));
            (void)class_slot(count, cls, t0 + k * NTH + tid < T);
        }
    }
    __syncthreads();
    if (tid == 0) {
        uint32_t acc = 0;
        for (int k = 0; k < 16; k++) { cursor[k] = acc; acc += count[k]; }
    }
    __syncthreads();
    for (int t0 = 0; t0 < T; t0 += 8 * NTH) {
        uint32_t len[8];
        uint2 rg[8];
#pragma unroll
        for (int k = 0; k < 8; k++) {
            const int t = t0 + k * NTH + tid;
            len[k] = t < T ? len_of(t) : 0u;
            rg[k] = (t < T && !empty_ranges) ? ranges[t] : make_uint2(0u, 0u);
        }
#pragma unroll
        for (int k = 0; k < 8; k++) {
            const int t = t0 + k * NTH + tid;
            const int cls = 15 - min(15, 32 - __clz((int)len[k]));
            const uint32_t at = class_slot(cursor, cls, t < T);
            if (t < T) {
                order[at] = (uint32_t)t;
                order_rec[at] = make_uint4((uint32_t)t, rg[k].x, rg[k].y, 0u);
            }
        }
    }
    for (int t = T + tid; t < Tpad; t += NTH) order[t] = 0xFFFFFFFFu;
    if (tid == 0) order[Tpad] = (uint32_t)T - count[15];
    if (tid == 0 && bg_state) {
        const uint32_t now[4] = {__float_as_uint(bg[0]), __float_as_uint(bg[1]), __float_as_uint(bg[2]), (uint32_t)normalize_depth};
        bg_state[4] = (now[0] != bg_state[0]) | (now[1] != bg_state[1]) | (now[2] != bg_state[2]) | (now[3] != bg_state[3]);
        bg_state[0] = now[0]; bg_state[1] = now[1]; bg_state[2] = now[2]; bg_state[3] = now[3];
    }
}

#endif

uint32_t higher_msb(uint32_t n);
size_t scan_temp_bytes(int32_t P);
size_t sort_temp_bytes(int64_t R);

int launch_preprocess(const SoarRastParams &prm, const float *means3D, const float *shs, const float *colors_precomp,
                      const float *opacities, const float *scales, const float *rotations, const float *cov3D_precomp,
                      GeomBuf &g, int32_t *radii, hipStream_t stream);
int launch_scan(const SoarRastParams &prm, GeomBuf &g, hipStream_t stream);
struct ZeroRange { void *ptr; size_t bytes; };
int launch_zero_ranges(const ZeroRange *ranges, int count, hipStream_t stream);
int launch_tile_order(const SoarRastParams &prm, ImageBuf &img, hipStream_t stream);

int launch_depth_buckets(const SoarRastParams &prm, GeomBuf &g, hipStream_t stream);
int launch_tile_binning(const SoarRastParams &prm, GeomBuf &g, BinBuf &b, ImageBuf &img, int64_t capacity, hipStream_t stream);
int launch_binning(const SoarRastParams &prm, GeomBuf &g, BinBuf &b, ImageBuf &img, int64_t R,
                   hipStream_t stream);
inline int blend_grid_ranks(int ntiles)
{
    const int r = (ntiles / 8 + 7) / 8 * 8;
    return r < 1024 ? 1024 : (r > 4096 ? 4096 : r);
}
int launch_block_masks(const SoarRastParams &prm, const GeomBuf &g, BinBuf &b, ImageBuf &img, int64_t R, hipStream_t stream);
int launch_tile_order_binned(const SoarRastParams &prm, const GeomBuf &g, BinBuf &b, ImageBuf &img, int64_t R, hipStream_t stream);

int launch_render_forward(const SoarRastParams &prm, const GeomBuf &g, const BinBuf &b, ImageBuf &img,
                          float *out_color, float *out_normal, float *out_depth, float *out_opac,
                          const float *occ_values, float *out_occ, hipStream_t stream);
int launch_occ_backward(const SoarRastParams &prm, const GeomBuf &g, const BinBuf &b, const ImageBuf &img, const float *dL_dout_occ,
                        float *dL_docc, hipStream_t stream);
int launch_render_backward(const SoarRastParams &prm, const GeomBuf &g, const BinBuf &b, const ImageBuf &img,
                           const float *dL_dcolor, const float *dL_dnormal, const float *dL_ddepth, const float *dL_dopac,
                           const float *grad_scale, float *acc, double *acc64, bool blend, const float *dL_dout_occ, float *dL_docc,
                           const float *normal_scale, int occ_planes, hipStream_t stream);
int launch_geometry_backward(const SoarRastParams &prm, const float *means3D, const int32_t *radii, const float *shs,
                             const float *scales, const float *rotations, const float *cov3D_precomp, const GeomBuf &g,
                             const float *acc, float *dL_dmeans2D, float *dL_dcolors, float *dL_dopacity,
                             float *dL_dmeans3D, float *dL_dcov3D, float *dL_dsh, float *dL_dscales, float *dL_drotations,
                             float *dL_dviewmat, float *dL_dprojmat, float *dL_dcampos, bool zero_camera_grads, hipStream_t stream,
                             float *dL_docc = nullptr);

}
```

### soar_amd/hip_lib.py

```python
from __future__ import annotations

import ctypes as C
import os
from typing import Optional

_HERE = os.path.dirname(os.path.abspath(__file__))
LIB_PATH = os.environ.get("SOAR_HIP_LIB") or os.path.join(_HERE, "_lib", "libsoar_hip.so")
if os.environ.get("SOAR_HIP_LIB"):
    import sys as _sys
    print(f"[soar_amd] SOAR_HIP_LIB is set: loading {LIB_PATH} instead of the in-tree build (development A/B runs only)", file=_sys.stderr)

FRAME_LOSS_SCRATCH_FLOATS = 4 * 2048
ABI_VERSION = 8
c_f32p = C.c_void_p
_vp = C.c_void_p


class SoarRastParams(C.Structure):
    _fields_ = [
        ("P", C.c_int32), ("W", C.c_int32), ("H", C.c_int32), ("sh_degree", C.c_int32), ("M", C.c_int32),
        ("prefiltered", C.c_int32), ("render_front", C.c_int32), ("sort_descending", C.c_int32), ("debug", C.c_int32),
        ("cfg_surface", C.c_int32), ("cfg_normalize_depth", C.c_int32), ("cfg_perpix_depth", C.c_int32),
        ("cfg_lrn_cam", C.c_int32),
        ("tanfovx", C.c_float), ("tanfovy", C.c_float), ("scale_modifier", C.c_float),
# ... 111 lines not shown
                ("small", C.c_float * DATA_SMALL_FLOATS),
                ("images", _vp), ("masks", _vp), ("normal_F", _vp), ("normal_B", _vp), ("normal_mask", _vp),
                ("rgb_crop", _vp), ("mask_crop", _vp), ("normal_Ks", _vp),
                ("rays_d", _vp), ("cam_d", _vp), ("gt_rays_d", _vp), ("gt_cam_d", _vp),
                ("gt_rgb", _vp), ("gt_mask", _vp), ("gt_normal_F", _vp), ("gt_normal_B", _vp), ("gt_normal_mask", _vp),
                ("gt_rgb_crop", _vp), ("gt_mask_crop", _vp),
                ("mvp_mtx", _vp), ("proj", _vp), ("gt_mvp_mtx", _vp), ("small_out", _vp)]


SIGNATURES = {
    "soar_last_error": (C.c_char_p, []),
    "soar_abi_version": (C.c_int, []),
    "soar_rast_geometry_bytes": (C.c_int, [C.c_int32, C.c_int32, C.POINTER(C.c_size_t)]),
    "soar_rast_image_bytes": (C.c_int, [C.c_int32, C.c_int32, C.POINTER(C.c_size_t)]),
    "soar_rast_binning_bytes": (C.c_int, [C.c_int64, C.POINTER(C.c_size_t)]),
    "soar_rast_backward_workspace_bytes": (C.c_int, [C.c_int32, C.POINTER(C.c_size_t)]),
    "soar_rast_forward_geometry": (C.c_int, [C.POINTER(SoarRastParams)] + [_vp] * 7 + [_vp, _vp, C.POINTER(C.c_int64), _vp]),
    "soar_rast_num_rendered": (C.c_int, [_vp, C.c_int32, C.c_int32, C.POINTER(C.c_int64), _vp]),
    "soar_rast_binning_status": (C.c_int, [_vp, C.c_int32, C.c_int32, C.POINTER(C.c_int64), C.POINTER(C.c_int64), _vp]),
    "soar_rast_binning_status_sticky": (C.c_int, [_vp, C.c_int32, C.c_int32, C.POINTER(C.c_int64), C.POINTER(C.c_int64), C.c_int32, _vp]),
    "soar_rast_binning_status_async": (C.c_int, [_vp, C.c_int32, C.c_int32, _vp, _vp]),
    "soar_rast_prefilter_violations": (C.c_int, [_vp, C.c_int32, C.c_int32, C.POINTER(C.c_int64), _vp]),
    "soar_rast_forward_render": (C.c_int, [C.POINTER(SoarRastParams), _vp, _vp, _vp, _vp, C.c_int64, _vp, _vp, _vp, _vp, _vp]),
    "soar_rast_forward_render_occ": (C.c_int, [C.POINTER(SoarRastParams), _vp, _vp, _vp, _vp, C.c_int64, _vp, _vp, _vp, _vp,
                                               _vp, _vp, _vp]),
    "soar_rast_backward": (C.c_int, [C.POINTER(SoarRastParams)] + [_vp] * 7 + [_vp, _vp, _vp, C.c_int64] + [_vp] * 4
                           + [_vp] * 11 + [_vp, C.c_size_t, _vp]),
    "soar_rast_backward_scaled": (C.c_int, [C.POINTER(SoarRastParams)] + [_vp] * 7 + [_vp, _vp, _vp, C.c_int64] + [_vp] * 5
                                  + [_vp] * 11 + [_vp, C.c_size_t, _vp]),
    "soar_rast_backward_occ": (C.c_int, [C.POINTER(SoarRastParams)] + [_vp] * 7 + [_vp, _vp, _vp, C.c_int64] + [_vp] * 6 + [C.c_int32]
                               + [_vp] * 12 + [_vp, C.c_size_t, _vp]),
    "soar_batch_begin": (C.c_int, [C.c_int32]),
    "soar_batch_frame": (C.c_int, [C.c_int32]),
    "soar_batch_end": (C.c_int, []),
    "soar_rast_occ_backward": (C.c_int, [C.POINTER(SoarRastParams), _vp, _vp, _vp, C.c_int64, _vp, _vp, _vp]),
    "soar_rast_mark_visible": (C.c_int, [C.c_int32, _vp, _vp, _vp, _vp, _vp]),
    "soar_rast_export_state": (C.c_int, [C.POINTER(SoarRastParams), _vp, _vp, _vp, C.c_int64] + [_vp] * 17 + [_vp]),
    "soar_lbs_knn_weights_bytes": (C.c_int, [C.c_int32, C.c_int32, C.POINTER(C.c_size_t)]),
    "soar_lbs_knn_weights": (C.c_int, [_vp, C.c_int32, _vp, C.c_int32, _vp, C.c_int32, C.c_int32, _vp, _vp, _vp, C.c_size_t, _vp]),
    "soar_lbs_knn_grid_bytes": (C.c_int, [C.c_int32, C.POINTER(C.c_size_t)]),
    "soar_lbs_knn_query_bytes": (C.c_int, [C.c_int32, C.POINTER(C.c_size_t)]),
    "soar_lbs_knn_build_grid": (C.c_int, [_vp, C.c_int32, _vp, C.c_int32, _vp, _vp]),
    "soar_lbs_knn_query": (C.c_int, [_vp, C.c_int32, _vp, C.c_int32, _vp, C.c_int32, C.c_int32, _vp, _vp, _vp, C.c_size_t, _vp]),
    "soar_lbs_knn_query_ordered": (C.c_int, [_vp, C.c_int32, _vp, C.c_int32, _vp, C.c_int32, C.c_int32, _vp, C.c_int32, _vp, _vp,
                                             _vp, C.c_size_t, _vp]),
    "soar_lbs_knn_state_bytes": (C.c_int, [C.c_int32, C.POINTER(C.c_size_t)]),
    "soar_lbs_knn_query_state": (C.c_int, [_vp, C.c_int32, _vp, C.c_int32, _vp, C.c_int32, _vp, C.c_int32, _vp, _vp, _vp, C.c_size_t, _vp]),
    "soar_lbs_knn_refresh": (C.c_int, [_vp, C.c_int32, C.c_int32, _vp, C.c_int32, _vp, _vp, _vp, _vp, _vp]),
    "soar_lbs_warp_forward": (C.c_int, [_vp] * 6 + [C.c_int32, C.c_int32] + [_vp] * 4),
    "soar_lbs_warp_backward": (C.c_int, [_vp] * 5 + [C.c_int32, C.c_int32] + [_vp] * 5),
    "soar_lbs_warp_forward_batch": (C.c_int, [_vp] * 4 + [C.c_int32] * 3 + [_vp] * 3),
    "soar_lbs_warp_backward_sum": (C.c_int, [_vp] * 4 + [C.c_int32] * 3 + [_vp] * 4 + [C.c_int32, _vp, _vp, _vp, _vp]),
    "soar_frames_warp_preprocess": (C.c_int, [C.c_int32, _vp] + [_vp] * 4 + [C.c_int32, C.c_int32] + [_vp] * 6),
    "soar_rast_backward_rows": (C.c_int, [_vp] * 22),
    "soar_frames_geometry_warp_backward": (C.c_int, [C.c_int32, _vp] + [_vp] * 4 + [C.c_int32, C.c_int32] + [_vp] * 7),
    "soar_dist2_knn3": (C.c_int, [_vp, C.c_int32, _vp, _vp]),
    "soar_depth2normal": (C.c_int, [C.c_int32, C.c_int32, _vp, _vp, C.c_float, C.c_float, C.c_float, C.c_float, _vp, _vp]),
    "soar_depth2normal_backward": (C.c_int, [C.c_int32, C.c_int32, _vp, _vp, C.c_float, C.c_float, C.c_float, C.c_float, _vp, _vp,
                                             _vp]),
    "soar_normal2curv": (C.c_int, [C.c_int32, C.c_int32, _vp, _vp, _vp, _vp]),
    "soar_normal2curv_backward": (C.c_int, [C.c_int32, C.c_int32, _vp, _vp, _vp, _vp, _vp]),
    "soar_view_finish": (C.c_int, [C.c_int32, C.c_int32, _vp, _vp, _vp, _vp, C.c_float, C.c_float, _vp, _vp, _vp, _vp]),
    "soar_view_finish_backward": (C.c_int, [C.c_int32, C.c_int32, _vp, _vp, _vp, _vp, C.c_float, C.c_float, _vp, _vp, _vp, _vp,
                                            _vp, _vp]),
    "soar_ssim_scratch_floats": (C.c_int, [C.c_int32, C.c_int32, C.c_int32, C.POINTER(C.c_size_t)]),
    "soar_ssim": (C.c_int, [C.c_int32, C.c_int32, C.c_int32, _vp, _vp, _vp, _vp, _vp, _vp]),
    "soar_ssim_rendered": (C.c_int, [C.c_int32, C.c_int32, C.c_int32, _vp, _vp, _vp, _vp, _vp, _vp, _vp]),
    "soar_densify_stats": (C.c_int, [C.c_int32, _vp, _vp, C.c_int32, _vp, _vp, _vp, _vp, _vp, _vp]),
    "soar_densify_plan_bytes": (C.c_int, [C.c_int32, C.POINTER(C.c_size_t)]),
    "soar_densify_plan": (C.c_int, [C.c_int32, _vp, _vp, _vp, C.c_int32, C.c_int32, C.c_float, C.c_float, C.c_float, C.c_float,
                                    C.c_float, _vp, C.POINTER(C.c_int64), _vp]),
    "soar_densify_flags": (C.c_int, [C.c_int32, _vp, _vp, _vp]),
    "soar_densify_apply": (C.c_int, [C.c_int32, C.c_int32, _vp, C.c_int32, C.POINTER(SoarDensifyRow), _vp, _vp, _vp, C.c_int32, _vp]),
    "soar_smplx_joint_mats": (C.c_int, [C.c_int32, C.c_int32, C.c_int32, _vp, C.c_int32, _vp, _vp, _vp, _vp, _vp, _vp, _vp, _vp]),
    "soar_image_loss_scratch_floats": (C.c_int, [C.POINTER(C.c_size_t)]),
    "soar_masked_l1": (C.c_int, [C.c_int32, C.c_int32, C.c_int32, _vp, _vp, _vp, _vp, _vp, _vp]),
    "soar_masked_l1_backward": (C.c_int, [C.c_int32, C.c_int32, C.c_int32, _vp, _vp, _vp, _vp, _vp, _vp, _vp]),
    "soar_cos_loss": (C.c_int, [C.c_int32, C.c_int32, C.c_int32, _vp, _vp, _vp, C.c_float, C.c_float, _vp, _vp, _vp]),
    "soar_cos_loss_backward": (C.c_int, [C.c_int32, C.c_int32, C.c_int32, _vp, _vp, _vp, C.c_float, C.c_float, _vp, _vp, _vp, _vp]),
    "soar_frame_loss": (C.c_int, [C.c_int32, C.c_int32, _vp, _vp, _vp, _vp, _vp, _vp, _vp, C.c_float, C.c_float, C.c_float,
                                  C.c_float, _vp, _vp, _vp, _vp, _vp, _vp, _vp, _vp, C.c_int32, _vp]),
    "soar_frame_loss_pooled": (C.c_int, [C.c_int32, C.c_int32, _vp, _vp, _vp, _vp, _vp, C.c_int32, _vp, C.c_float, C.c_float, C.c_float,
                                         C.c_float, _vp, _vp, _vp, _vp, _vp, _vp, _vp, _vp, C.c_int32, _vp]),
    "soar_selftest_exp": (C.c_int, [_vp, C.c_int32, _vp, _vp, _vp]),
    "soar_selftest_affine_scan": (C.c_int, [_vp, _vp, _vp, _vp]),
    "soar_prof_enable": (C.c_int, [C.c_int]),
    "soar_prof_reset": (C.c_int, []),
    "soar_prof_stage_count": (C.c_int, []),
    "soar_prof_stage_name": (C.c_char_p, [C.c_int]),
    "soar_prof_read": (C.c_int, [C.c_int, C.POINTER(C.c_double), C.POINTER(C.c_int64)]),
    "soar_sum_frames": (C.c_int, [C.c_int32, C.c_int64, _vp, _vp, _vp]),
    "soar_gather_step_inputs": (C.c_int, [C.c_int32, C.c_int32, C.c_int32, C.c_int32, _vp, _vp, _vp, _vp, _vp]),
    "soar_gather_step_inputs_ids": (C.c_int, [C.c_int32, C.c_int32, C.c_int32, C.c_int32, C.POINTER(C.c_int32), _vp, _vp, _vp, _vp]),
    "soar_prof_timestamp": (C.c_int, [_vp, C.c_int64, C.c_int64, _vp]),
    "soar_view_buffer_bytes": (C.c_int, [C.c_int32, C.c_int32, C.c_int32, C.c_int64, C.c_int32, C.POINTER(C.c_size_t)]),
    "soar_views_grad_scratch_floats": (C.c_int, [C.c_int32, C.c_int32, C.POINTER(C.c_size_t)]),
    "soar_views_forward": (C.c_int, [C.POINTER(SoarPoseArgs), C.c_int32, C.POINTER(SoarViewArgs), _vp]),
    "soar_views_backward": (C.c_int, [C.POINTER(SoarPoseArgs), C.c_int32, C.POINTER(SoarViewArgs), _vp]),
    "soar_step_views_forward": (C.c_int, [C.c_int32, C.POINTER(SoarPoseArgs), C.POINTER(C.c_int32), C.POINTER(SoarViewArgs), _vp]),
    "soar_step_views_backward": (C.c_int, [C.c_int32, C.POINTER(SoarPoseArgs), C.POINTER(C.c_int32), C.POINTER(SoarViewArgs), _vp]),
    "soar_cameras_from_c2w": (C.c_int, [C.c_int32, _vp, C.POINTER(C.c_float), C.POINTER(SoarCameraSpec), _vp, _vp]),
    "soar_rast_forward_render_status": (C.c_int, [C.POINTER(SoarRastParams), _vp, _vp, _vp, _vp, C.c_int64, _vp, _vp, _vp, _vp,
                                                  _vp, _vp, _vp, _vp]),
    "soar_lbs_warp_backward_views": (C.c_int, [_vp] * 5 + [C.c_int32] * 3 + [_vp] * 4 + [C.c_int32, _vp, _vp, _vp, _vp]),
    "soar_avatar_loss_scratch_floats": (C.c_int, [C.POINTER(C.c_size_t)]),
    "soar_avatar_pixel_losses": (C.c_int, [C.POINTER(SoarAvatarLossArgs), C.c_int32, _vp]),
    "soar_adam_step": (C.c_int, [C.c_int32, C.POINTER(SoarAdamRow), C.c_double, C.c_double, C.c_double, _vp, _vp]),
    "soar_adam_step_at": (C.c_int, [C.c_int32, C.POINTER(SoarAdamRow), C.c_double, C.c_double, C.c_double, C.c_int64, _vp]),
    "soar_adam_step_rows": (C.c_int, [C.c_int32, C.POINTER(SoarAdamRow), C.c_double, C.c_double, C.c_double, _vp, C.c_int32, _vp]),
    "soar_adam_step_rows_wide": (C.c_int, [C.c_int32, C.POINTER(SoarAdamRow), C.c_double, C.c_double, C.c_double, _vp, C.c_int32, _vp]),
    "soar_tsdf_integrate": (C.c_int, [C.c_int32] * 3 + [_vp] * 5 + [C.c_float] * 4 + [C.c_int32] * 3 + [C.c_float] * 3 + [_vp] * 3),
    "soar_mc_workspace_bytes": (C.c_int, [C.c_int32] * 3 + [C.POINTER(C.c_size_t)]),
    "soar_mc_count": (C.c_int, [C.c_int32] * 3 + [_vp, _vp, C.c_float, _vp, C.c_size_t, C.POINTER(C.c_int64), _vp]),
    "soar_mc_emit": (C.c_int, [C.c_int32] * 3 + [_vp, _vp, C.c_float, _vp, C.c_size_t, _vp, _vp, _vp]),
    "soar_mesh_filter_bytes": (C.c_int, [C.c_int32, C.c_int32, C.POINTER(C.c_size_t)]),
    "soar_mesh_filter_components": (C.c_int, [C.c_int32, C.c_int32, _vp, _vp, C.c_int32, C.c_float, _vp, C.c_size_t, _vp, _vp,
                                              C.POINTER(C.c_int64), _vp]),
    "soar_field_workspace_bytes": (C.c_int, [C.c_int32, C.POINTER(C.c_size_t)]),
    "soar_field_forward": (C.c_int, [C.POINTER(SoarFieldArgs), _vp]),
    "soar_field_backward": (C.c_int, [C.POINTER(SoarFieldArgs), _vp, C.c_size_t, _vp]),
    "soar_envmap_workspace_bytes": (C.c_int, [C.c_int32, C.c_int32, C.c_int32, C.POINTER(C.c_size_t)]),
    "soar_envmap_forward": (C.c_int, [C.POINTER(SoarEnvmapArgs), _vp]),
    "soar_envmap_backward": (C.c_int, [C.POINTER(SoarEnvmapArgs), _vp, C.c_size_t, _vp]),
    "soar_lpips_weights_bytes": (C.c_int, [C.POINTER(C.c_size_t)]),
    "soar_lpips_pack_weights": (C.c_int, [C.POINTER(SoarLpipsWeights), _vp, C.c_size_t, _vp]),
    "soar_lpips_workspace_bytes": (C.c_int, [C.c_int32, C.c_int32, C.c_int32, C.c_int32, C.POINTER(C.c_size_t)]),
    "soar_lpips_forward": (C.c_int, [C.POINTER(SoarLpipsArgs), _vp, C.c_size_t, _vp]),
    "soar_lpips_backward": (C.c_int, [C.POINTER(SoarLpipsArgs), _vp, C.c_size_t, _vp]),
    "soar_vae_weights_floats": (C.c_int, [C.POINTER(C.c_size_t)]),
    "soar_vae_weights_bytes": (C.c_int, [C.POINTER(C.c_size_t)]),
    "soar_vae_pack_weights": (C.c_int, [_vp, C.c_size_t, _vp, C.c_size_t, _vp]),
    "soar_vae_workspace_bytes": (C.c_int, [C.c_int32, C.c_int32, C.c_int32, C.c_int32, C.POINTER(C.c_size_t)]),
    "soar_vae_forward": (C.c_int, [C.POINTER(SoarVaeArgs), _vp, C.c_size_t, _vp]),
    "soar_vae_backward": (C.c_int, [C.POINTER(SoarVaeArgs), _vp, C.c_size_t, _vp]),
    "soar_sds_q_sample": (C.c_int, [C.POINTER(SoarSdsArgs), _vp]),
    "soar_sds_loss": (C.c_int, [C.POINTER(SoarSdsArgs), _vp]),
    "soar_surfel_activations_forward": (C.c_int, [C.c_int32, C.c_int32] + [_vp] * 10 + [_vp]),
    "soar_surfel_activations_backward": (C.c_int, [C.c_int32, C.c_int32] + [_vp] * 16 + [_vp]),
    "soar_surfel_regularizers_workspace_bytes": (C.c_int, [C.c_int32, C.POINTER(C.c_size_t)]),
    "soar_surfel_regularizers": (C.c_int, [C.c_int32] * 3 + [_vp] * 11 + [_vp, C.c_size_t, _vp]),
    "soar_smplx_vertices": (C.c_int, [C.c_int32] * 4 + [_vp, C.c_int32] + [_vp] * 8 + [_vp]),
    "soar_mesh_workspace_bytes": (C.c_int, [C.c_int32, C.POINTER(C.c_size_t)]),
    "soar_mesh_subdivide_edges": (C.c_int, [C.c_int32, C.c_int32, _vp, _vp, C.c_size_t, C.POINTER(C.c_int64), _vp]),
    "soar_mesh_subdivide": (C.c_int, [C.c_int32, C.c_int32, C.c_int64, _vp, _vp, _vp, C.c_size_t, _vp, _vp, _vp]),
    "soar_mesh_vertex_normals": (C.c_int, [C.c_int32, C.c_int32, _vp, _vp, C.c_int32, _vp, C.c_size_t, _vp, _vp]),
    "soar_mesh_vertex_frames": (C.c_int, [C.c_int32, _vp, _vp, _vp, _vp]),
    "soar_data_mask_bbox": (C.c_int, [C.c_int32, C.c_int32, C.c_int32, _vp, _vp, _vp]),
    "soar_data_crops": (C.c_int, [C.c_int32, C.c_int32, C.c_int32, _vp, _vp, _vp, _vp, _vp, _vp]),
    "soar_data_step_batch": (C.c_int, [C.POINTER(SoarDataStepArgs), _vp]),
}

_lib: Optional[C.CDLL] = None


class SoarHipError(RuntimeError):
    pass


def lib() -> C.CDLL:
    global _lib
    if _lib is None:
        import torch
        if not os.path.exists(LIB_PATH):
            raise SoarHipError(
                f"{LIB_PATH} not found: the HIP extension is not built. Run `python -m soar_amd.build` "
                "(hipcc --offload-arch=gfx950). soar_amd has no CPU fallback.")
        handle = C.CDLL(LIB_PATH)
        for name, (res, args) in SIGNATURES.items():
            fn = getattr(handle, name)
            fn.restype = res
            fn.argtypes = args
        if handle.soar_abi_version() != ABI_VERSION:
            raise SoarHipError("libsoar_hip.so ABI version mismatch; rebuild with `python -m soar_amd.build --force`")
        _lib = handle
    return _lib

# ... 16 lines not shown
```

### soar_amd/step_plan.py

```python
from __future__ import annotations

import ctypes as C
import os
from typing import Dict, List, Optional, Sequence

import torch

from . import hip_lib
from .hip_lib import check, ptr
from .rasterizer import _Ctx


class FrameStepPlan:
    def __init__(self, seq, n_frames: int, targets: Dict[str, torch.Tensor], bg: torch.Tensor, capacity: int, flat,
                 loss_weights: Sequence[float] = (1.0, 1.0, 0.1, 0.01), use_graphs: bool = True, batched: Optional[bool] = None,
                 loss: str = "synthetic", lambdas: Optional[Dict[str, float]] = None):
        if loss not in ("synthetic", "avatar"):
            raise ValueError(f"loss must be 'synthetic' or 'avatar', got {loss!r}")
        self.loss_kind = loss
        if loss == "avatar" and (use_graphs or not torch.is_tensor(targets)):
            raise ValueError("loss='avatar' needs a resident target pool and use_graphs=False")
        L = hip_lib.lib()
        self.L, self.seq, self.flat, self.n = L, seq, flat, int(n_frames)
        dev = seq.device
# ... 8 lines not shown
            if targets.dim() != 4 or targets.shape[1:] != (7, H, W) or not targets.is_cuda or not targets.is_contiguous():
                raise ValueError(f"target pool must be a contiguous device tensor [n_sets,7,{H},{W}], got {tuple(targets.shape)}")
            self.pool = targets
            self.targets = None
        else:
            self.targets = [targets[k].to(**f).contiguous() for k in ("color", "mask", "normal")]
        self.frame_sel = torch.zeros((self.n,), dtype=torch.int32, device=dev)
        self.frame_ids = torch.zeros((self.n,), dtype=torch.int32, device=dev)
        self._ids_pinned = torch.zeros((64, self.n), dtype=torch.int32).pin_memory()
        self._ids_copied = [None] * 64
        self.mats = torch.empty((self.n, 55, 4, 4), **f)
        self.blend_weights = torch.empty((P, seq.lbs_weights.shape[1]), **f)
        self.ones = torch.ones((P, 1), **f)
        self.ctx = _Ctx(P, 0, H, W, seq.camera.tanfovx, seq.camera.tanfovy, 1.0, 0, False, False, False, False, self.bg,
                        seq.view, seq.proj, seq.prcp, seq.patch, seq.campos, seq.config, dev)
        nbytes = C.c_size_t(0)
        check(L.soar_rast_geometry_bytes(P, 0, C.byref(nbytes)), "geometry_bytes"); geom_b = nbytes.value
        check(L.soar_rast_image_bytes(W, H, C.byref(nbytes)), "image_bytes"); img_b = nbytes.value
        check(L.soar_rast_binning_bytes(self.capacity, C.byref(nbytes)), "binning_bytes"); bin_b = nbytes.value
        check(L.soar_rast_backward_workspace_bytes(P, C.byref(nbytes)), "workspace_bytes"); work_b = nbytes.value
        u8 = dict(dtype=torch.uint8, device=dev)
        self.xyz_p_all, self.rot_p_all = torch.empty((self.n, P, 3), **f), torch.empty((self.n, P, 4), **f)
        self.g_means3D_all, self.g_rot_p_all = torch.empty((self.n, P, 3), **f), torch.empty((self.n, P, 4), **f)
        self.views: List[dict] = []
        for i in range(self.n):
            v = dict(
                xyz_p=self.xyz_p_all[i], rot_p=self.rot_p_all[i], radii=torch.empty((P,), dtype=torch.int32, device=dev),
                color=torch.empty((3, H, W), **f), normal=torch.empty((3, H, W), **f), depth=torch.empty((1, H, W), **f),
                opac=torch.empty((1, H, W), **f), occ=torch.empty((3, H, W), **f),
                geom=torch.empty(geom_b, **u8), img=torch.empty(img_b, **u8), binning=torch.empty(bin_b, **u8),
                work=torch.empty(work_b, **u8), loss=torch.empty((), **f), sums=torch.empty((hip_lib.FRAME_LOSS_SCRATCH_FLOATS,), **f),
                gC=torch.empty((3, H, W), **f), gN=torch.empty((3, H, W), **f), gD=torch.empty((1, H, W), **f),
                gO=torch.empty((1, H, W), **f),
                g_means2D=torch.empty((P, 3), **f), g_colors=torch.empty((P, 3), **f), g_opacity=torch.empty((P, 1), **f),
                g_means3D=self.g_means3D_all[i], g_cov3D=torch.empty((P, 6), **f), g_scales=torch.empty((P, 3), **f),
                g_rot_p=self.g_rot_p_all[i], g_view=torch.empty((4, 4), **f), g_proj=torch.empty((4, 4), **f),
                g_campos=torch.empty((3,), **f))
            v["geom"][:256].zero_()
            self.views.append(v)
        self.fused_tail = os.environ.get("SOAR_PLAN_FUSED_TAIL", "1") != "0" and self.n <= 8
        if self.fused_tail:
            self.ctx.params.debug |= 8
            self._tail_frames = (hip_lib.SoarFrameTail * self.n)()
            for i, v in enumerate(self.views):
                t = self._tail_frames[i]
                t.prm = C.addressof(self.ctx.params)
                t.means3D, t.rotations, t.radii = v["xyz_p"].data_ptr(), v["rot_p"].data_ptr(), v["radii"].data_ptr()
                t.geom_buffer, t.workspace, t.dL_dmeans2D = v["geom"].data_ptr(), v["work"].data_ptr(), v["g_means2D"].data_ptr()
        self.fused_head = os.environ.get("SOAR_PLAN_FUSED_HEAD", "1") != "0" and self.n <= 8
        if self.fused_head:
            self.ctx.params.debug |= 16
            self._head_frames = (hip_lib.SoarFrameHead * self.n)()
            for i, v in enumerate(self.views):
                h = self._head_frames[i]
                h.prm, h.geom_buffer, h.radii = C.addressof(self.ctx.params), v["geom"].data_ptr(), v["radii"].data_ptr()
        self.g_xyz = torch.empty((self.n, P, 3), **f)
        self.g_rot = torch.empty((self.n, P, 4), **f)
        self.g_scales = torch.empty((self.n, P, 3), **f)
        self.g_colors = torch.empty((self.n, P, 3), **f)
        self.losses = torch.empty((self.n,), **f)
        from . import lbs as _lbs
        self.knn = _lbs.KnnFollower(seq.knn_grid, P)
        for name in ("opacity", "occ"):
            if name in flat.views:
                flat.views[name].zero_()
        if loss == "avatar":
            self._setup_avatar(lambdas)
        self.steps = 0
        self.STAMP_CAP = 8192
        self.stamps = torch.zeros((1 + 2 * self.STAMP_CAP,), dtype=torch.int64, device=dev) if os.environ.get("SOAR_PLAN_TIMESTAMPS") in ("1", "2") else None
        self.fine_stamps = os.environ.get("SOAR_PLAN_TIMESTAMPS") == "2"
        self.stale = None
        self._baked = self._leaf_signature()
        self.streams = [torch.cuda.Stream(device=dev) for _ in range(self.n)]
        if batched is None:
            env = os.environ.get("SOAR_PLAN_BATCHED")
            batched = (env != "0") if env in ("0", "1") else (self.W * self.H <= 3_000_000)
        self.batched = bool(batched) and self.n <= 8
        self._call_cache = {}
        self.optimizer = None
        self.optimizer_in_two_parts = None
        self.graphs = None
        self._ids_by_value = not use_graphs and self.n <= 8
        if use_graphs:
            if os.environ.get("DEBUG_CLR_GRAPH_PACKET_CAPTURE") != "0":
                raise RuntimeError("FrameStepPlan(use_graphs=True) needs DEBUG_CLR_GRAPH_PACKET_CAPTURE=0 in the environment "
                                   "before the HIP runtime starts (see the module docstring); use use_graphs=False otherwise")
            self._capture()

    def _setup_avatar(self, lambdas):
        from .losses import _AvatarStageLoss as S
        L, dev, H, W, P = self.L, self.device, self.H, self.W, self.P
        f = dict(dtype=torch.float32, device=dev)
        lam = dict(recon=1.0, mask=1.0, normal=1.0, occ=0.1)
        lam.update(lambdas or {})
        self.lam = lam
        pool = self.pool
        n_sets = int(pool.shape[0])
        m = pool[:, 3:4]
        self.av = dict(rgb=pool[:, 0:3], mask=m, normal=pool[:, 4:7],
                       sel=(m > 1e-5).reshape(n_sets, H, W).contiguous().view(torch.uint8),
                       sel_occ=(m > 0).reshape(n_sets, H, W).contiguous().view(torch.uint8),
                       blended=(pool[:, 0:3] * m + self.bg.reshape(1, 3, 1, 1) * (1 - m)).contiguous())
        k = C.c_size_t(0)
        check(L.soar_image_loss_scratch_floats(C.byref(k)), "soar_image_loss_scratch_floats")
        n_loss = int(k.value)
        check(L.soar_ssim_scratch_floats(3, H, W, C.byref(k)), "soar_ssim_scratch_floats")
        n_ssim = int(k.value)
        coef = [0.0] * S.N
        coef[S.L1], coef[S.SSIM], coef[S.ONE] = 0.8 * lam["recon"], -0.2 * lam["recon"], 0.2 * lam["recon"]
        coef[S.L1M], coef[S.COS] = lam["mask"], 0.2 * lam["normal"]
        self.av_coef = torch.tensor(coef, **f)
        self.av_occ_up = torch.tensor([lam["occ"]], **f)
        self.av_counts = torch.stack([self.av["sel"].reshape(n_sets, -1).sum(1).float(), torch.full((n_sets,), float(H * W), **f),
                                      torch.zeros((n_sets,), **f), self.av["sel_occ"].reshape(n_sets, -1).sum(1).float()], dim=1).contiguous()
        self.av_cos_scale_all = torch.zeros((self.n,), **f)
        check(L.soar_avatar_loss_scratch_floats(C.byref(k)), "soar_avatar_loss_scratch_floats")
        n_pix = int(k.value)
        self._av_args = {}
        self.av_focal = (H / (2.0 * self.seq.camera.tanfovy), W / (2.0 * self.seq.camera.tanfovx))
        self.g_occ_all = torch.empty((self.n, P), **f)
        self.av_gC_all, self.av_g_ssim_all = torch.empty((self.n, 3, H, W), **f), torch.empty((self.n, 3, H, W), **f)
        self.av_terms_all, self.av_occ_terms_all = torch.zeros((self.n, S.N), **f), torch.zeros((self.n, 2), **f)
        self.av_terms_all[:, S.ONE] = 1.0
        for i, v in enumerate(self.views):
            g_nd = torch.zeros((4, H, W), **f)
            v.update(normal_out=torch.empty((3, H, W), **f), curv=torch.empty((1, H, W), **f), pred=torch.empty((3, H, W), **f),
                     gC=self.av_gC_all[i], g_ssim=self.av_g_ssim_all[i], g_nd=g_nd,
                     g_occ_img=torch.empty((3, H, W), **f), terms=self.av_terms_all[i], occ_terms=self.av_occ_terms_all[i],
                     av_scratch=torch.empty((max(n_loss, n_ssim),), **f), av_pix_scratch=torch.empty((n_pix,), **f))
            v["gN"], v["gD"] = g_nd[:3], g_nd[3:]

    def _av(self, i: int):
        from .losses import _AvatarStageLoss as S
        v = self.views[i]
        k = self._frames_now[i] % int(self.pool.shape[0])
        at = lambda t, j: t.data_ptr() + 4 * j
        return S, self.L, v, self.W, self.H, self.av, k, at, ptr(v["av_scratch"]), v["terms"], self.av_coef

    def _av_finish(self, i, stream):
        S, L, v, W, H, a, k, at, sc, t, up = self._av(i)
        check(L.soar_view_finish(W, H, ptr(v["normal"]), ptr(v["depth"]), ptr(v["opac"]), ptr(self.ctx.keep[3]), self.av_focal[0],
                                 self.av_focal[1], ptr(v["normal_out"]), ptr(v["curv"]), ptr(v["pred"]), stream), "soar_view_finish")

    def _av_ssim(self, i, stream):
        S, L, v, W, H, a, k, at, sc, t, up = self._av(i)
        check(L.soar_ssim_rendered(3, H, W, ptr(v["color"]), ptr(a["blended"][k]), at(t, S.SSIM), sc, ptr(v["g_ssim"]), ptr(v["opac"]), stream),
              "soar_ssim_rendered")

    def _av_pixel_args(self, i):
        S, L, v, W, H, a, k, at, sc, t, up = self._av(i)
        return hip_lib.SoarAvatarLossArgs(
            H=H, W=W, cos_limit=1.0, cos_weight=1.0, render=ptr(v["color"]), gt_rgb=ptr(a["rgb"][k]), mask_img=ptr(v["opac"]),
            gt_mask=ptr(a["mask"][k]), normal=ptr(v["normal_out"]), gt_normal=ptr(a["normal"][k]), occ=ptr(v["occ"]),
            sel=ptr(a["sel"][k]), sel_normal=ptr(a["sel"][k]), sel_occ=ptr(a["sel_occ"][k]), stats=at(t, S.L1), stats_occ=ptr(v["occ_terms"]),
            scratch=ptr(v["av_pix_scratch"]), counts=ptr(self.av_counts[k]), up_l1=at(up, S.L1), up_l1m=at(up, S.L1M), up_cos=at(up, S.COS),
            up_occ=ptr(self.av_occ_up), up_ssim=at(up, S.SSIM), g_ssim=ptr(v["g_ssim"]), g_render=ptr(v["gC"]), g_mask=ptr(v["gO"]),
            g_normal=ptr(v["gN"]), g_occ=ptr(v["g_occ_img"]), normal_raw=1, occ_grad_summed=1, cos_scale_out=self.av_cos_scale_all.data_ptr() + 4 * i,
            background=self.ctx.params.bg_dev)

    def _av_pixel(self, i, stream):
        key = ("av_pixel", i, self._frames_now[i] % int(self.pool.shape[0]))
        args = self._av_args.get(key)
        if args is None:
            args = self._av_args[key] = self._av_pixel_args(i)
        check(self.L.soar_avatar_pixel_losses(C.byref(args), 3, stream), "soar_avatar_pixel_losses")

    def _f_avatar_loss(self, i: int, frame: int, stream: int) -> None:
        v, up = self.views[i], self.av_coef
        for stage in (self._av_finish, self._av_ssim, self._av_pixel):
            stage(i, stream)
        torch.add(torch.dot(v["terms"], up), v["occ_terms"][0] * self.av_occ_up[0], out=self.losses[i])

    def _leaf_signature(self):
        s = self.seq
        return tuple((t.data_ptr(), tuple(t.shape)) for t in (s.xyz, s.rot, s.scales, s.colors, s.occ))

    def invalidate(self, reason: str):
        self.stale = reason

    def _check_fresh(self):
        if self.stale is None and self._leaf_signature() != self._baked:
            self.stale = "the sequence's parameter tensors changed (pointer or shape) since the plan was built"
        if self.stale is not None:
            raise RuntimeError(f"FrameStepPlan is stale: {self.stale}; build a new plan (buffers and HIP graphs hold the old "
                               "pointers)")

    RESORT_EVERY = 1024

    def _stamp(self, k: int, stream: int) -> None:
        if self.stamps is not None:
            check(self.L.soar_prof_timestamp(self.stamps.data_ptr(), self.STAMP_CAP, k, stream), "timestamp")

    def _stage_stamp(self, i: int, stage: int, stream: int) -> None:
        if self.stamps is not None and self.fine_stamps:
            self._stamp(100 + 10 * i + stage, stream)

    def _prologue(self, stream: int, resort: bool = True) -> None:
        L, s = self.L, self.seq
        self._stamp(0, stream)
        n_sets = int(self.pool.shape[0]) if self.pool is not None else 0
        if self._ids_by_value:
            ids = (C.c_int32 * self.n)(*self._frames_now)
            check(L.soar_gather_step_inputs_ids(self.n, s.num_frames, 55 * 16, n_sets, ids, ptr(s.cano2live), ptr(self.mats),
                                                ptr(self.frame_sel), stream), "gather_step_inputs")
        else:
            check(L.soar_gather_step_inputs(self.n, s.num_frames, 55 * 16, n_sets, ptr(self.frame_ids), ptr(s.cano2live), ptr(self.mats),
                                            ptr(self.frame_sel), stream), "gather_step_inputs")
        if resort:
            self.knn.full(s.xyz.detach(), self.blend_weights, stream)
        else:
            self.knn.calls = 1
            self.knn.refresh(s.xyz.detach(), self.blend_weights, stream)
        self._stamp(1, stream)

    def _warp_all(self, stream: int) -> None:
        L, s = self.L, self.seq
        J = int(self.blend_weights.shape[1])
        if self.fused_head:
            check(L.soar_frames_warp_preprocess(self.n, self._head_frames, ptr(s.xyz.detach()), ptr(s.rot.detach()), ptr(self.blend_weights),
                                                ptr(self.mats), self.P, J, ptr(s.colors.detach()), ptr(self.ones), ptr(s.scales.detach()),
                                                ptr(self.xyz_p_all), ptr(self.rot_p_all), stream), "frames_warp_preprocess")
            return
        check(L.soar_lbs_warp_forward_batch(ptr(s.xyz.detach()), ptr(s.rot.detach()), ptr(self.blend_weights), ptr(self.mats), self.n,
                                            self.P, J, ptr(self.xyz_p_all), ptr(self.rot_p_all), stream), "warp_forward_batch")

    def _call(self, key, build) -> None:
        c = self._call_cache.get(key)
        if c is None:
            c = self._call_cache[key] = build()
        if c[0](*c[1]) != 0:
            check(1, c[2])

    def _f_geometry(self, i: int, stream: int) -> None:
        def build():
            L, s, v = self.L, self.seq, self.views[i]
            return (L.soar_rast_forward_geometry, (C.byref(self.ctx.params), ptr(v["xyz_p"]), None, ptr(s.colors.detach()), ptr(self.ones),
                                                   ptr(s.scales.detach()), ptr(v["rot_p"]), None, ptr(v["geom"]), ptr(v["radii"]), None, stream),
                    "geometry")
        self._call(("geometry", i, stream), build)

    def _f_render(self, i: int, stream: int) -> None:
        def build():
            L, s, v = self.L, self.seq, self.views[i]
            return (L.soar_rast_forward_render_occ, (C.byref(self.ctx.params), ptr(v["radii"]), ptr(v["geom"]), ptr(v["binning"]), ptr(v["img"]),
                                                     self.capacity, ptr(v["color"]), ptr(v["normal"]), ptr(v["depth"]), ptr(v["opac"]),
                                                     ptr(s.occ), ptr(v["occ"]), stream), "render")
        self._call(("render", i, stream), build)

    def _f_loss(self, i: int, stream: int) -> None:
        def build():
            L, v, W, H = self.L, self.views[i], self.W, self.H
            wc, wm, wn, wd = self.weights
            if self.pool is not None:
                return (L.soar_frame_loss_pooled, (W, H, ptr(v["color"]), ptr(v["normal"]), ptr(v["depth"]), ptr(v["opac"]), ptr(self.pool),
                                                   int(self.pool.shape[0]), ptr(self.frame_sel[i]), wc, wm, wn, wd, ptr(self.losses[i]),
                                                   ptr(v["sums"]), ptr(v["gC"]), ptr(v["gN"]), ptr(v["gD"]), ptr(v["gO"]), ptr(v["img"]),
                                                   self.ctx.params.bg_dev, int(self.ctx.params.cfg_normalize_depth), stream),
                        "frame_loss_pooled")
            tc, tm, tn = self.targets
            return (L.soar_frame_loss, (W, H, ptr(v["color"]), ptr(v["normal"]), ptr(v["depth"]), ptr(v["opac"]), ptr(tc), ptr(tm), ptr(tn),
                                        wc, wm, wn, wd, ptr(self.losses[i]), ptr(v["sums"]), ptr(v["gC"]), ptr(v["gN"]), ptr(v["gD"]),
                                        ptr(v["gO"]), ptr(v["img"]), self.ctx.params.bg_dev, int(self.ctx.params.cfg_normalize_depth), stream),
                    "frame_loss")
        self._call(("loss", i, stream), build)

    def _f_backward(self, i: int, stream: int) -> None:
        def build():
            L, s, v = self.L, self.seq, self.views[i]
            return (L.soar_rast_backward, (C.byref(self.ctx.params), ptr(v["xyz_p"]), ptr(v["radii"]), None, ptr(s.colors.detach()),
                                           ptr(s.scales.detach()), ptr(v["rot_p"]), None, ptr(v["geom"]), ptr(v["binning"]), ptr(v["img"]),
                                           self.capacity, ptr(v["gC"]), ptr(v["gN"]), ptr(v["gD"]), ptr(v["gO"]), ptr(v["g_means2D"]),
                                           ptr(self.g_colors[i]), ptr(v["g_opacity"]), ptr(v["g_means3D"]), ptr(v["g_cov3D"]), None,
                                           ptr(self.g_scales[i]), ptr(v["g_rot_p"]), ptr(v["g_view"]), ptr(v["g_proj"]), ptr(v["g_campos"]),
                                           ptr(v["work"]), v["work"].numel(), stream), "backward")
        self._call(("backward", i, stream), build)

    def _f_backward_occ(self, i: int, stream: int) -> None:
        def build():
            L, s, v = self.L, self.seq, self.views[i]
            return (L.soar_rast_backward_occ, (C.byref(self.ctx.params), ptr(v["xyz_p"]), ptr(v["radii"]), None, ptr(s.colors.detach()),
                                               ptr(s.scales.detach()), ptr(v["rot_p"]), None, ptr(v["geom"]), ptr(v["binning"]), ptr(v["img"]),
                                               self.capacity, ptr(v["gC"]), ptr(v["gN"]), ptr(v["gD"]), ptr(v["gO"]), ptr(v["g_occ_img"]),
                                               self.av_cos_scale_all.data_ptr() + 4 * i, 1, ptr(v["g_means2D"]), ptr(self.g_colors[i]), ptr(v["g_opacity"]), ptr(v["g_means3D"]),
                                               ptr(v["g_cov3D"]), None, ptr(self.g_scales[i]), ptr(v["g_rot_p"]), ptr(v["g_view"]),
                                               ptr(v["g_proj"]), ptr(v["g_campos"]), ptr(self.g_occ_all[i]), ptr(v["work"]), v["work"].numel(),
                                               stream), "backward_occ")
        self._call(("backward_occ", i, stream), build)

    def _frame(self, i: int, stream: int) -> None:
        self._stamp(2 + 2 * i, stream)
        if self.loss_kind == "avatar":
            self._f_geometry(i, stream)
            self._f_render(i, stream)
            self._f_avatar_loss(i, self._frames_now[i], stream)
            self._f_backward_occ(i, stream)
            self._stamp(3 + 2 * i, stream)
            return
        for k, stage in enumerate((self._f_geometry, self._f_render, self._f_loss, self._f_backward)):
            self._stage_stamp(i, k, stream)
            stage(i, stream)
        self._stage_stamp(i, 4, stream)
        self._stamp(3 + 2 * i, stream)

    def _frames_batched(self, stream: int, frames: Optional[Sequence[int]] = None) -> None:
        L = self.L
        frames = list(range(self.n)) if frames is None else list(frames)
        for i in frames:
            self._stamp(2 + 2 * i, stream)
        def batch(stages):
            check(L.soar_batch_begin(len(frames)), "batch_begin")
            try:
                for stage in stages:
                    for k, i in enumerate(frames):
                        check(L.soar_batch_frame(k), "batch_frame")
                        stage(i, stream)
            finally:
                L.soar_batch_end()
        if self.loss_kind == "avatar":
            from .losses import _AvatarStageLoss as S
            batch((self._f_geometry, self._f_render, self._av_finish, self._av_ssim, self._av_pixel, self._f_backward_occ))
            if len(frames) == self.n:
                torch.addmv(self.av_occ_terms_all[:, 0] * self.av_occ_up[0], self.av_terms_all, self.av_coef, out=self.losses)
            else:
                for i in frames:
                    v = self.views[i]
                    torch.add(torch.dot(v["terms"], self.av_coef), v["occ_terms"][0] * self.av_occ_up[0], out=self.losses[i])
        else:
            batch((self._f_geometry, self._f_render, self._f_loss, self._f_backward))
        for i in frames:
            self._stamp(3 + 2 * i, stream)

    def _epilogue(self, stream: int) -> None:
        L, s = self.L, self.seq
        self._stamp(2 * self.n + 2, stream)
        J = int(self.blend_weights.shape[1])
        fv = self.flat.views
        src = (C.c_void_p * 2)(ptr(self.g_scales), ptr(self.g_colors))
        dst = (C.c_void_p * 2)(ptr(fv["scales"]), ptr(fv["colors"]))
        width = (C.c_int32 * 2)(3, 3)
        if self.fused_tail:
            occ = ptr(fv["occ"]) if (self.loss_kind == "avatar" and "occ" in fv) else None
            check(L.soar_frames_geometry_warp_backward(self.n, self._tail_frames, ptr(s.xyz.detach()), ptr(s.rot.detach()), ptr(self.blend_weights),
                                                       ptr(self.mats), self.P, J, ptr(s.scales.detach()), ptr(fv["xyz"]), ptr(fv["rot"]),
                                                       ptr(fv["scales"]), ptr(fv["colors"]), occ, stream), "frames_geometry_warp_backward")
            self._stamp(2 * self.n + 3, stream)
            return
        check(L.soar_lbs_warp_backward_sum(ptr(s.xyz.detach()), ptr(s.rot.detach()), ptr(self.blend_weights), ptr(self.mats), self.n,
                                           self.P, J, ptr(self.g_means3D_all), ptr(self.g_rot_p_all), ptr(fv["xyz"]), ptr(fv["rot"]),
                                           2, src, dst, width, stream), "warp_backward_sum")
        if self.loss_kind == "avatar" and "occ" in fv:
            check(L.soar_sum_frames(self.n, self.P, ptr(self.g_occ_all), ptr(fv["occ"]), stream), "sum_frames")
        self._stamp(2 * self.n + 3, stream)

    def _capture(self) -> None:
        dev = self.device
        self.frame_ids.copy_(torch.arange(self.n, dtype=torch.int32) % max(self.seq.num_frames, 1))
        self._run_eager()
        torch.cuda.synchronize(dev)
        cap = torch.cuda.Stream(device=dev)
        graphs = {}
        with torch.cuda.device(dev):
            for name, resort in (("prologue_resort", True), ("prologue", False)):
                g = torch.cuda.CUDAGraph()
                with torch.cuda.graph(g, stream=cap):
                    self._prologue(cap.cuda_stream, resort)
                graphs[name] = g
                g = torch.cuda.CUDAGraph()
                with torch.cuda.graph(g, stream=cap):
                    self._prologue(cap.cuda_stream, resort)
                    self._warp_all(cap.cuda_stream)
                graphs[name + "+warp"] = g
            for i in range(self.n):
                g = torch.cuda.CUDAGraph()
                with torch.cuda.graph(g, stream=cap):
                    self._frame(i, cap.cuda_stream)
                graphs[i] = g
            for name, fn in (("warp", self._warp_all), ("epilogue", self._epilogue)):
                g = torch.cuda.CUDAGraph()
                with torch.cuda.graph(g, stream=cap):
                    fn(cap.cuda_stream)
                graphs[name] = g
        torch.cuda.synchronize(dev)
        self.graphs = graphs

    def _run_eager(self) -> None:
        dev = self.device
        main = torch.cuda.current_stream(dev)
        with torch.cuda.device(dev):
            opt = self.optimizer if (self.optimizer is not None and self.steps > 0) else None
            in_flight = any(p is not None for p in self.flat.pending) if self.optimizer_in_two_parts is None else self.optimizer_in_two_parts
            in_flight = in_flight and self.flat.n_buckets > 1
            self.flat.wait_bucket(0)
            if opt is not None:
                opt.step(main.cuda_stream, names=("xyz",) if in_flight else None, advance=True)
            self._prologue(main.cuda_stream, self.steps % self.RESORT_EVERY == 0)
            self.flat.wait_all()
            if opt is not None and in_flight:
                opt.step(main.cuda_stream, names=tuple(n for n in opt.names if n != "xyz"), advance=False)
            self._warp_all(main.cuda_stream)
            if self.batched:
                self._frames_batched(main.cuda_stream)
            else:
                self._fan_out(main, lambda i, s: self._frame(i, s.cuda_stream))
            self._epilogue(main.cuda_stream)
        self.steps += 1
        self.ctx.params.debug |= 4

    def _fan_out(self, main, fn) -> None:
        ev = torch.cuda.Event()
        ev.record(main)
        done = []
# ... 60 lines not shown
```

Baseline: 5257.

## Fold loss-finish and step-gather kernels into neighboring launches to cut launch count

The single-block loss-finish reduction is deferred and run as an extra block inside the backward zero-ranges kernel. The per-step input gather is parked and run as extra blocks of the KNN kernels, so two small kernel launches per frame or step disappear. This targets launch and dispatch overhead between dependent stages. In exchange it adds host-side parked state per batch slot, extra branches at the top of hot kernels, and risk if a parked launch is never consumed or flushed on the right stream.

```diff
diff --git a/include/soar_hip.h b/include/soar_hip.h
--- a/include/soar_hip.h
+++ b/include/soar_hip.h
@@ -214,6 +214,18 @@
                            float w_color, float w_mask, float w_normal, float w_depth, float *loss_out, float *scratch,
                            float *dL_dcolor, float *dL_dnormal, float *dL_ddepth, float *dL_dopac, const void *image_buffer,
                            const float *background, int32_t normalize_depth, void *stream);
+
+int soar_frame_loss_fused_finish(int32_t W, int32_t H, const float *color, const float *normal, const float *depth,
+                                 const float *opac, const float *target_color, const float *target_mask,
+                                 const float *target_normal, float w_color, float w_mask, float w_normal, float w_depth,
+                                 float *loss_out, float *scratch, float *dL_dcolor, float *dL_dnormal, float *dL_ddepth,
+                                 float *dL_dopac, const void *image_buffer, const float *background, int32_t normalize_depth,
+                                 void *stream);
+int soar_frame_loss_pooled_fused_finish(int32_t W, int32_t H, const float *color, const float *normal, const float *depth,
+                                        const float *opac, const float *target_pool, int32_t n_sets, const int32_t *set_index_dev,
+                                        float w_color, float w_mask, float w_normal, float w_depth, float *loss_out, float *scratch,
+                                        float *dL_dcolor, float *dL_dnormal, float *dL_ddepth, float *dL_dopac,
+                                        const void *image_buffer, const float *background, int32_t normalize_depth, void *stream);
 
 typedef struct SoarAvatarLossArgs {
     int32_t H, W;
@@ -354,6 +366,9 @@
 int soar_gather_step_inputs_ids(int32_t n_frames, int32_t num_frames_seq, int32_t floats_per_frame, int32_t n_sets,
                                 const int32_t *frame_ids_host, const float *table_dev, float *mats_out_dev,
                                 int32_t *set_index_out_dev, void *stream);
+int soar_gather_step_inputs_ids_fused(int32_t n_frames, int32_t num_frames_seq, int32_t floats_per_frame, int32_t n_sets,
+                                      const int32_t *frame_ids_host, const float *table_dev, float *mats_out_dev,
+                                      int32_t *set_index_out_dev, void *stream);
 
 typedef struct SoarAdamRow {
     float *param;
diff --git a/soar_amd/csrc/api.hip b/soar_amd/csrc/api.hip
--- a/soar_amd/csrc/api.hip
+++ b/soar_amd/csrc/api.hip
@@ -44,16 +44,26 @@
 
 namespace {
 constexpr int ZERO_RANGES = 5;
-struct ZeroArgs { uint32_t *ptr[ZERO_RANGES]; size_t words[ZERO_RANGES]; size_t first_block[ZERO_RANGES + 1]; };
+struct ZeroArgs {
+    uint32_t *ptr[ZERO_RANGES]; size_t words[ZERO_RANGES]; size_t first_block[ZERO_RANGES + 1];
+    LossFinishArgs finish;
+};
 constexpr int ZERO_UNROLL = 8;
 constexpr size_t ZERO_BLOCK_WORDS = 256 * 4 * ZERO_UNROLL;
 __global__ void __launch_bounds__(256) zero_ranges_kernel(Batch<ZeroArgs> b)
 {
     const ZeroArgs &z = b.v[blockIdx.y];
-    if (blockIdx.x >= z.first_block[ZERO_RANGES]) return;
+    const unsigned rider = z.finish.loss ? 1u : 0u;
+    if (rider && blockIdx.x == 0) {
+        __shared__ float4 red[256];
+        loss_finish_block(z.finish, red);
+        return;
+    }
+    const size_t bx = blockIdx.x - rider;
+    if (bx >= z.first_block[ZERO_RANGES]) return;
     int r = 0;
-    while (r < ZERO_RANGES - 1 && blockIdx.x >= z.first_block[r + 1]) r++;
-    const size_t b0 = ((size_t)blockIdx.x - z.first_block[r]) * ZERO_BLOCK_WORDS;
+    while (r < ZERO_RANGES - 1 && bx >= z.first_block[r + 1]) r++;
+    const size_t b0 = (bx - z.first_block[r]) * ZERO_BLOCK_WORDS;
     uint32_t *p = z.ptr[r];
     const size_t n = z.words[r];
     if (b0 + ZERO_BLOCK_WORDS <= n && (reinterpret_cast<uintptr_t>(p) & 15) == 0) {
@@ -66,9 +76,10 @@
 }
 }
 
-int launch_zero_ranges(const ZeroRange *ranges, int count, hipStream_t stream)
+int launch_zero_ranges(const ZeroRange *ranges, int count, hipStream_t stream, const LossFinishArgs *finish)
 {
     ZeroArgs z;
+    z.finish = finish ? *finish : LossFinishArgs{nullptr, 0, 0, 0.f, 0.f, 0.f, 0.f, nullptr};
     size_t blocks = 0;
     if (count > ZERO_RANGES) { set_error("launch_zero_ranges: at most %d ranges", ZERO_RANGES); return 1; }
     for (int r = 0; r < ZERO_RANGES; r++) {
@@ -78,6 +89,7 @@
         blocks += (z.words[r] + ZERO_BLOCK_WORDS - 1) / ZERO_BLOCK_WORDS;
     }
     z.first_block[ZERO_RANGES] = blocks;
+    if (finish) blocks++;
     if (blocks == 0) return 0;
     SOAR_LAUNCH_BATCHED(zero_ranges_kernel, dim3((unsigned)blocks), dim3(256), 0, stream, z);
     return post_launch("zero_ranges", stream, 0);
@@ -690,7 +702,9 @@
     {
         const ZeroRange zr[4] = {{wide ? (void *)acc64 : (void *)acc, (wide ? sizeof(double) : sizeof(float)) * ACC_STRIDE * (size_t)prm->P},
                                  {dL_dviewmat, 16 * sizeof(float)}, {dL_dprojmat, 16 * sizeof(float)}, {dL_dcampos, 3 * sizeof(float)}};
-        if (launch_zero_ranges(zr, 4, stream)) return 1;
+        LossFinishArgs fin;
+        const bool ride = take_loss_finish(stream, &fin);
+        if (launch_zero_ranges(zr, 4, stream, ride ? &fin : nullptr)) return 1;
     }
     if (num_rendered > 0 || wide) {
         if (launch_render_backward(*prm, g, b, img, dL_dout_color, dL_dout_normal, dL_dout_depth, dL_dout_opac, grad_scale_dev, acc,
diff --git a/soar_amd/csrc/frame_loss.hip b/soar_amd/csrc/frame_loss.hip
--- a/soar_amd/csrc/frame_loss.hip
+++ b/soar_amd/csrc/frame_loss.hip
@@ -104,40 +104,10 @@
         a.sums[4 * blockIdx.x + threadIdx.x] = (part[0][threadIdx.x] + part[1][threadIdx.x]) + (part[2][threadIdx.x] + part[3][threadIdx.x]);
 }
 
-struct LossFinishArgs {
-    const float *sums;
-    int blocks, n;
-    float wc, wm, wn, wd;
-    float *loss;
-};
 __global__ void __launch_bounds__(256) frame_loss_finish_kernel(Batch<LossFinishArgs> batch)
 {
-    const LossFinishArgs &fa = batch.v[blockIdx.y];
-    const float *sums = fa.sums;
-    const int blocks = fa.blocks, n = fa.n;
-    const float wc = fa.wc, wm = fa.wm, wn = fa.wn, wd = fa.wd;
-    float *loss = fa.loss;
     __shared__ float4 red[256];
-    float4 acc = make_float4(0.f, 0.f, 0.f, 0.f);
-    for (int b = threadIdx.x; b < blocks; b += 256) {
-        const float4 v = reinterpret_cast<const float4 *>(sums)[b];
-        acc.x += v.x; acc.y += v.y; acc.z += v.z; acc.w += v.w;
-    }
-    red[threadIdx.x] = acc;
-    __syncthreads();
-    for (int off = 128; off > 0; off >>= 1) {
-        if ((int)threadIdx.x < off) {
-            const float4 o = red[threadIdx.x + off];
-            float4 m = red[threadIdx.x];
-            m.x += o.x; m.y += o.y; m.z += o.z; m.w += o.w;
-            red[threadIdx.x] = m;
-        }
-        __syncthreads();
-    }
-    if (threadIdx.x == 0) {
-        const float4 S = red[0];
-        *loss = (wc * S.x / (3.f * n) + wm * S.y / n) + (wn * S.z / (3.f * n) + wd * S.w / n);
-    }
+    loss_finish_block(batch.v[blockIdx.y], red);
 }
 
 }
@@ -150,7 +120,8 @@
                              const float *target_color, const float *target_mask, const float *target_normal,
                              const int32_t *set_index_dev, int32_t n_sets, float w_color, float w_mask, float w_normal,
                              float w_depth, float *loss_out, float *sums4, float *dL_dcolor, float *dL_dnormal, float *dL_ddepth,
-                             float *dL_dopac, const void *image_buffer, const float *background, int32_t normalize_depth, hipStream_t stream);
+                             float *dL_dopac, const void *image_buffer, const float *background, int32_t normalize_depth, hipStream_t stream,
+                             bool park_finish = false);
 
 extern "C" int soar_frame_loss(int32_t W, int32_t H, const float *color, const float *normal, const float *depth,
                                const float *opac, const float *target_color, const float *target_mask,
@@ -181,7 +152,8 @@
                              const float *target_color, const float *target_mask, const float *target_normal,
                              const int32_t *set_index_dev, int32_t n_sets, float w_color, float w_mask, float w_normal,
                              float w_depth, float *loss_out, float *sums4, float *dL_dcolor, float *dL_dnormal, float *dL_ddepth,
-                             float *dL_dopac, const void *image_buffer, const float *background, int32_t normalize_depth, hipStream_t stream)
+                             float *dL_dopac, const void *image_buffer, const float *background, int32_t normalize_depth, hipStream_t stream,
+                             bool park_finish)
 {
     if (W <= 0 || H <= 0) { set_error("soar_frame_loss: bad image size %dx%d", W, H); return 1; }
     if (!color || !normal || !depth || !opac || !target_color || !target_mask || !target_normal || !loss_out || !sums4 ||
@@ -212,10 +184,102 @@
     const int blocks = min(SOAR_FRAME_LOSS_SCRATCH_FLOATS / 4, max(1, (a.n / (vec4 ? 4 : 1) + 255) / 256));
     if (vec4) SOAR_LAUNCH_BATCHED(frame_loss_kernel<4>, dim3(blocks), dim3(256), 0, stream, a);
     else SOAR_LAUNCH_BATCHED(frame_loss_kernel<1>, dim3(blocks), dim3(256), 0, stream, a);
-    const soar::LossFinishArgs fa = {sums4, blocks, a.n, w_color, w_mask, w_normal, w_depth, loss_out};
+    const LossFinishArgs fa = {sums4, blocks, a.n, w_color, w_mask, w_normal, w_depth, loss_out};
+    if (park_finish) {
+        SOAR_LAUNCH_OK("frame_loss", stream, 0);
+        return park_loss_finish(fa, stream);
+    }
     SOAR_LAUNCH_BATCHED(frame_loss_finish_kernel, dim3(1), dim3(256), 0, stream, fa);
     SOAR_LAUNCH_OK("frame_loss", stream, 0);
     return 0;
+}
+
+extern "C" int soar_frame_loss_fused_finish(int32_t W, int32_t H, const float *color, const float *normal, const float *depth,
+                                            const float *opac, const float *target_color, const float *target_mask,
+                                            const float *target_normal, float w_color, float w_mask, float w_normal, float w_depth,
+                                            float *loss_out, float *sums4, float *dL_dcolor, float *dL_dnormal, float *dL_ddepth,
+                                            float *dL_dopac, const void *image_buffer, const float *background, int32_t normalize_depth,
+                                            void *stream_)
+{
+    return frame_loss_launch(W, H, color, normal, depth, opac, target_color, target_mask, target_normal, nullptr, 1, w_color,
+                             w_mask, w_normal, w_depth, loss_out, sums4, dL_dcolor, dL_dnormal, dL_ddepth, dL_dopac, image_buffer,
+                             background, normalize_depth, static_cast<hipStream_t>(stream_), true);
+}
+
+extern "C" int soar_frame_loss_pooled_fused_finish(int32_t W, int32_t H, const float *color, const float *normal, const float *depth,
+                                                   const float *opac, const float *target_pool, int32_t n_sets,
+                                                   const int32_t *set_index_dev, float w_color, float w_mask, float w_normal,
+                                                   float w_depth, float *loss_out, float *sums4, float *dL_dcolor, float *dL_dnormal,
+                                                   float *dL_ddepth, float *dL_dopac, const void *image_buffer, const float *background,
+                                                   int32_t normalize_depth, void *stream_)
+{
+    if (n_sets <= 0 || !set_index_dev) { set_error("soar_frame_loss_pooled_fused_finish: need n_sets > 0 and a device index"); return 1; }
+    return frame_loss_launch(W, H, color, normal, depth, opac, target_pool, target_pool, target_pool, set_index_dev, n_sets,
+                             w_color, w_mask, w_normal, w_depth, loss_out, sums4, dL_dcolor, dL_dnormal, dL_ddepth, dL_dopac,
+                             image_buffer, background, normalize_depth, static_cast<hipStream_t>(stream_), true);
+}
+
+namespace soar {
+namespace {
+struct ParkedLoss { bool valid; hipStream_t stream; LossFinishArgs fa; };
+struct ParkedGather { bool valid; hipStream_t stream; StepGatherArgs ga; };
+thread_local ParkedLoss g_parked_loss[MAX_BATCH];
+thread_local ParkedGather g_parked_gather;
+__global__ void __launch_bounds__(256) frame_loss_finish_one_kernel(LossFinishArgs fa)
+{
+    __shared__ float4 red[256];
+    loss_finish_block(fa, red);
+}
+__global__ void gather_step_inputs_parked_kernel(StepGatherArgs ga) { step_gather_block(ga, blockIdx.x); }
+}
+
+int park_loss_finish(const LossFinishArgs &fa, hipStream_t stream)
+{
+    const BatchCtx &c = batch_ctx();
+    ParkedLoss &p = g_parked_loss[c.n ? c.f : 0];
+    if (p.valid) {
+        p.valid = false;
+        hipLaunchKernelGGL(frame_loss_finish_one_kernel, dim3(1), dim3(256), 0, p.stream, p.fa);
+        if (post_launch("frame_loss_finish", p.stream, 0)) return 1;
+    }
+    p.valid = true; p.stream = stream; p.fa = fa;
+    return 0;
+}
+
+bool take_loss_finish(hipStream_t stream, LossFinishArgs *out)
+{
+    const BatchCtx &c = batch_ctx();
+    ParkedLoss &p = g_parked_loss[c.n ? c.f : 0];
+    if (!p.valid || p.stream != stream) return false;
+    p.valid = false;
+    *out = p.fa;
+    return true;
+}
+
+int flush_step_gather()
+{
+    ParkedGather &p = g_parked_gather;
+    if (!p.valid) return 0;
+    p.valid = false;
+    hipLaunchKernelGGL(gather_step_inputs_parked_kernel, dim3(p.ga.n_frames), dim3(256), 0, p.stream, p.ga);
+    return post_launch("gather_step_inputs", p.stream, 0);
+}
+
+int park_step_gather(const StepGatherArgs &ga, hipStream_t stream)
+{
+    if (flush_step_gather()) return 1;
+    g_parked_gather.valid = true; g_parked_gather.stream = stream; g_parked_gather.ga = ga;
+    return 0;
+}
+
+bool take_step_gather(hipStream_t stream, StepGatherArgs *out)
+{
+    ParkedGather &p = g_parked_gather;
+    if (!p.valid || p.stream != stream) return false;
+    p.valid = false;
+    *out = p.ga;
+    return true;
+}
 }
 
 
@@ -308,3 +372,19 @@
     SOAR_LAUNCH_OK("gather_step_inputs", stream, 0);
     return 0;
 }
+
+extern "C" int soar_gather_step_inputs_ids_fused(int32_t n_frames, int32_t num_frames_seq, int32_t floats_per_frame, int32_t n_sets,
+                                                 const int32_t *frame_ids_host, const float *table_dev, float *mats_out_dev,
+                                                 int32_t *set_index_out_dev, void *stream_)
+{
+    using namespace soar;
+    if (n_frames <= 0 || n_frames > MAX_BATCH || num_frames_seq <= 0 || floats_per_frame <= 0 || !frame_ids_host || !table_dev || !mats_out_dev) {
+        set_error("soar_gather_step_inputs_ids_fused: bad arguments (at most %d frames per step)", MAX_BATCH);
+        return 1;
+    }
+    StepGatherArgs ga = {};
+    ga.n_frames = n_frames; ga.num_frames_seq = num_frames_seq; ga.floats_per_frame = floats_per_frame; ga.n_sets = n_sets;
+    for (int f = 0; f < n_frames; f++) ga.id[f] = frame_ids_host[f];
+    ga.table = table_dev; ga.mats_out = mats_out_dev; ga.set_out = set_index_out_dev;
+    return park_step_gather(ga, static_cast<hipStream_t>(stream_));
+}
diff --git a/soar_amd/csrc/lbs_knn.hip b/soar_amd/csrc/lbs_knn.hip
--- a/soar_amd/csrc/lbs_knn.hip
+++ b/soar_amd/csrc/lbs_knn.hip
@@ -442,9 +442,10 @@
                 const uint32_t *__restrict__ q_keys, const uint32_t *__restrict__ q_ids,
                 const float *__restrict__ rows_padded, int J, float *__restrict__ weights_out,
                 int32_t *__restrict__ knn_idx_out, const uint32_t *__restrict__ item_order,
-                KnnStatePtrs state)
+                KnnStatePtrs state, StepGatherArgs gather)
 {
     constexpr int K = KNN_K;
+    if (blockIdx.x >= gridDim.x - (uint32_t)gather.n_frames) { step_gather_block(gather, (int)(blockIdx.x - (gridDim.x - (uint32_t)gather.n_frames))); return; }
     __shared__ float4 cand[KNN_CAND];
     __shared__ uint32_t row_start[KNN_ROWS], row_prefix[KNN_ROWS + 1];
     __shared__ int info[4];
@@ -455,7 +456,7 @@
     __shared__ float list_w[KNN_WAVES][WAVE];
 
     const int wave = threadIdx.x >> 6, lane = threadIdx.x & 63;
-    const uint32_t n_items = gridDim.x;
+    const uint32_t n_items = gridDim.x - (uint32_t)gather.n_frames;
     const bool ordered = item_order && item_order[n_items] == (KNN_ORDER_STAMP ^ n_items);
     const uint32_t n_chunks = n_items / KNN_SLOTS;
     const uint32_t item = ordered ? min(item_order[blockIdx.x], n_items - 1u) : (blockIdx.x % n_chunks) * KNN_SLOTS + blockIdx.x / n_chunks;
@@ -739,10 +740,11 @@
 constexpr int KNN_CERT_PAIRS = SOAR_KNN_CERT_PAIRS;
 __global__ void __launch_bounds__(KNN_WAVES *WAVE)
 knn_certify_kernel(const float *__restrict__ xyz, int P, const float4 *__restrict__ sorted_verts, const uint32_t *__restrict__ order,
-                   KnnStatePtrs st)
-{
+                   KnnStatePtrs st, StepGatherArgs gather)
+{
+    if ((int)blockIdx.x < gather.n_frames) { step_gather_block(gather, (int)blockIdx.x); return; }
     const int wave = threadIdx.x >> 6, lane = threadIdx.x & 63, l5 = lane & (KNN_KEEP - 1);
-    const int q_base = ((int)blockIdx.x * KNN_WAVES + wave) * (2 * KNN_CERT_PAIRS) + (lane >> 5);
+    const int q_base = (((int)blockIdx.x - gather.n_frames) * KNN_WAVES + wave) * (2 * KNN_CERT_PAIRS) + (lane >> 5);
     if (q_base - (lane >> 5) >= P) return;
     int qs[KNN_CERT_PAIRS];
     float4 ra[KNN_CERT_PAIRS], rb[KNN_CERT_PAIRS], vv[KNN_CERT_PAIRS];
@@ -1177,13 +1179,15 @@
         hipLaunchKernelGGL(item_cost_kernel, dim3(nchunks), dim3(WAVE), 0, stream, qk1, P, g.meta, g.cell_range, ws.item_cost);
         hipLaunchKernelGGL(item_order_kernel, dim3(1), dim3(1024), 0, stream, ws.item_cost, nchunks * KNN_SLOTS, ws.item_order);
     }
-    const dim3 grid(((P + WAVE - 1) / WAVE) * KNN_SLOTS);
+    StepGatherArgs gather = {};
+    if (state) (void)take_step_gather(stream, &gather);
+    const dim3 grid(((P + WAVE - 1) / WAVE) * KNN_SLOTS + gather.n_frames);
     if (knn_idx_out)
         hipLaunchKernelGGL(knn_cell_kernel<true>, grid, dim3(KNN_WAVES * WAVE), 0, stream, xyz, P, V, g.meta, g.cell_range,
-                           g.sorted_verts, qk1, qv1, g.rows, J, weights_out, knn_idx_out, ws.item_order, st);
+                           g.sorted_verts, qk1, qv1, g.rows, J, weights_out, knn_idx_out, ws.item_order, st, gather);
     else
         hipLaunchKernelGGL(knn_cell_kernel<false>, grid, dim3(KNN_WAVES * WAVE), 0, stream, xyz, P, V, g.meta, g.cell_range,
-                           g.sorted_verts, qk1, qv1, g.rows, J, weights_out, knn_idx_out, ws.item_order, st);
+                           g.sorted_verts, qk1, qv1, g.rows, J, weights_out, knn_idx_out, ws.item_order, st, gather);
     SOAR_LAUNCH_OK("lbs_knn_weights", stream, 0);
     return 0;
 }
@@ -1281,7 +1285,7 @@
     hipStream_t stream = static_cast<hipStream_t>(stream_);
     if (check_knn_sizes(P, V, J, KNN_K)) return 1;
     if (V < KNN_STATE_STRIDE) { set_error("soar_lbs_knn_query_state: the neighbour state keeps %d vertices per query, V=%d", KNN_STATE_STRIDE, V); return 1; }
-    if (P == 0) return 0;
+    if (P == 0) return flush_step_gather();
     if (!grid_buffer || !xyz || !vert_weights || !weights_out || !order || !state_buffer) { set_error("soar_lbs_knn_query_state: NULL pointer"); return 1; }
     if (check_ws("soar_lbs_knn_query_state", query_workspace, query_workspace_bytes) || check_ws("soar_lbs_knn_query_state", state_buffer, 0)) return 1;
     KnnGrid g;
@@ -1302,7 +1306,7 @@
     if (check_knn_sizes(P, V, J, KNN_K)) return 1;
     if (J > KNN_JMAX) { set_error("soar_lbs_knn_refresh: J <= %d", KNN_JMAX); return 1; }
     if (V < KNN_STATE_STRIDE) { set_error("soar_lbs_knn_refresh: the neighbour state keeps %d vertices per query, V=%d", KNN_STATE_STRIDE, V); return 1; }
-    if (P == 0) return 0;
+    if (P == 0) return flush_step_gather();
     if (!grid_buffer || !xyz || !weights_out || !state_buffer || !order) { set_error("soar_lbs_knn_refresh: NULL pointer"); return 1; }
     if (check_ws("soar_lbs_knn_refresh", state_buffer, 0)) return 1;
     KnnGrid g;
@@ -1312,7 +1316,10 @@
     StageTimer timer(ST_LBS_KNN, stream);
     const int per_block = KNN_WAVES * 2 * KNN_CERT_PAIRS, nblocks = (P + per_block - 1) / per_block;
     static_assert(SOAR_KNN_SEARCH_BLOCKS * KNN_WAVES % KNN_WORK_LISTS == 0, "searchers per list");
-    hipLaunchKernelGGL(knn_certify_kernel, dim3(nblocks), dim3(KNN_WAVES * WAVE), 0, stream, xyz, P, g.sorted_verts, order, st.p);
+    StepGatherArgs gather = {};
+    (void)take_step_gather(stream, &gather);
+    hipLaunchKernelGGL(knn_certify_kernel, dim3(nblocks + gather.n_frames), dim3(KNN_WAVES * WAVE), 0, stream, xyz, P, g.sorted_verts, order,
+                       st.p, gather);
     const int search_blocks = SOAR_KNN_SEARCH_BLOCKS, blend_blocks = (P + KNN_WAVES * KNN_FSLOTS - 1) / (KNN_WAVES * KNN_FSLOTS);
     hipLaunchKernelGGL(knn_blend_search_kernel, dim3(search_blocks + blend_blocks), dim3(KNN_WAVES * WAVE), 0, stream, xyz, P, search_blocks,
                        g.meta, g.cell_range, g.sorted_verts, g.rows, J, order, st.p, weights_out, searched_counter_dev);
diff --git a/soar_amd/csrc/soar_common.h b/soar_amd/csrc/soar_common.h
--- a/soar_amd/csrc/soar_common.h
+++ b/soar_amd/csrc/soar_common.h
@@ -327,6 +327,61 @@
 
 #endif
 
+struct LossFinishArgs {
+    const float *sums;
+    int blocks, n;
+    float wc, wm, wn, wd;
+    float *loss;
+};
+struct StepGatherArgs {
+    int n_frames, num_frames_seq, floats_per_frame, n_sets;
+    int32_t id[MAX_BATCH];
+    const float *table;
+    float *mats_out;
+    int32_t *set_out;
+};
+#if defined(__HIPCC__)
+static __device__ __forceinline__ void loss_finish_block(const LossFinishArgs &fa, float4 *red)
+{
+    const float *sums = fa.sums;
+    const int blocks = fa.blocks, n = fa.n;
+    const float wc = fa.wc, wm = fa.wm, wn = fa.wn, wd = fa.wd;
+    float4 acc = make_float4(0.f, 0.f, 0.f, 0.f);
+    for (int b = threadIdx.x; b < blocks; b += 256) {
+        const float4 v = reinterpret_cast<const float4 *>(sums)[b];
+        acc.x += v.x; acc.y += v.y; acc.z += v.z; acc.w += v.w;
+    }
+    red[threadIdx.x] = acc;
+    __syncthreads();
+    for (int off = 128; off > 0; off >>= 1) {
+        if ((int)threadIdx.x < off) {
+            const float4 o = red[threadIdx.x + off];
+            float4 m = red[threadIdx.x];
+            m.x += o.x; m.y += o.y; m.z += o.z; m.w += o.w;
+            red[threadIdx.x] = m;
+        }
+        __syncthreads();
+    }
+    if (threadIdx.x == 0) {
+        const float4 S = red[0];
+        *fa.loss = (wc * S.x / (3.f * n) + wm * S.y / n) + (wn * S.z / (3.f * n) + wd * S.w / n);
+    }
+}
+static __device__ __forceinline__ void step_gather_block(const StepGatherArgs &ga, int f)
+{
+    int id = ga.id[f] % ga.num_frames_seq;
+    if (id < 0) id += ga.num_frames_seq;
+    for (int k = threadIdx.x; k < ga.floats_per_frame; k += blockDim.x)
+        ga.mats_out[(size_t)f * ga.floats_per_frame + k] = ga.table[(size_t)id * ga.floats_per_frame + k];
+    if (threadIdx.x == 0 && ga.set_out) ga.set_out[f] = ga.n_sets > 0 ? id % ga.n_sets : 0;
+}
+#endif
+int park_loss_finish(const LossFinishArgs &fa, hipStream_t stream);
+bool take_loss_finish(hipStream_t stream, LossFinishArgs *out);
+int park_step_gather(const StepGatherArgs &ga, hipStream_t stream);
+bool take_step_gather(hipStream_t stream, StepGatherArgs *out);
+int flush_step_gather();
+
 uint32_t higher_msb(uint32_t n);
 size_t scan_temp_bytes(int32_t P);
 size_t sort_temp_bytes(int64_t R);
@@ -336,7 +391,7 @@
                       GeomBuf &g, int32_t *radii, hipStream_t stream);
 int launch_scan(const SoarRastParams &prm, GeomBuf &g, hipStream_t stream);
 struct ZeroRange { void *ptr; size_t bytes; };
-int launch_zero_ranges(const ZeroRange *ranges, int count, hipStream_t stream);
+int launch_zero_ranges(const ZeroRange *ranges, int count, hipStream_t stream, const LossFinishArgs *finish = nullptr);
 int launch_tile_order(const SoarRastParams &prm, ImageBuf &img, hipStream_t stream);
 
 int launch_depth_buckets(const SoarRastParams &prm, GeomBuf &g, hipStream_t stream);
diff --git a/soar_amd/hip_lib.py b/soar_amd/hip_lib.py
--- a/soar_amd/hip_lib.py
+++ b/soar_amd/hip_lib.py
@@ -217,6 +217,10 @@
                                   C.c_float, _vp, _vp, _vp, _vp, _vp, _vp, _vp, _vp, C.c_int32, _vp]),
     "soar_frame_loss_pooled": (C.c_int, [C.c_int32, C.c_int32, _vp, _vp, _vp, _vp, _vp, C.c_int32, _vp, C.c_float, C.c_float, C.c_float,
                                          C.c_float, _vp, _vp, _vp, _vp, _vp, _vp, _vp, _vp, C.c_int32, _vp]),
+    "soar_frame_loss_fused_finish": (C.c_int, [C.c_int32, C.c_int32, _vp, _vp, _vp, _vp, _vp, _vp, _vp, C.c_float, C.c_float, C.c_float,
+                                               C.c_float, _vp, _vp, _vp, _vp, _vp, _vp, _vp, _vp, C.c_int32, _vp]),
+    "soar_frame_loss_pooled_fused_finish": (C.c_int, [C.c_int32, C.c_int32, _vp, _vp, _vp, _vp, _vp, C.c_int32, _vp, C.c_float, C.c_float,
+                                                      C.c_float, C.c_float, _vp, _vp, _vp, _vp, _vp, _vp, _vp, _vp, C.c_int32, _vp]),
     "soar_selftest_exp": (C.c_int, [_vp, C.c_int32, _vp, _vp, _vp]),
     "soar_selftest_affine_scan": (C.c_int, [_vp, _vp, _vp, _vp]),
     "soar_prof_enable": (C.c_int, [C.c_int]),
@@ -227,6 +231,7 @@
     "soar_sum_frames": (C.c_int, [C.c_int32, C.c_int64, _vp, _vp, _vp]),
     "soar_gather_step_inputs": (C.c_int, [C.c_int32, C.c_int32, C.c_int32, C.c_int32, _vp, _vp, _vp, _vp, _vp]),
     "soar_gather_step_inputs_ids": (C.c_int, [C.c_int32, C.c_int32, C.c_int32, C.c_int32, C.POINTER(C.c_int32), _vp, _vp, _vp, _vp]),
+    "soar_gather_step_inputs_ids_fused": (C.c_int, [C.c_int32, C.c_int32, C.c_int32, C.c_int32, C.POINTER(C.c_int32), _vp, _vp, _vp, _vp]),
     "soar_prof_timestamp": (C.c_int, [_vp, C.c_int64, C.c_int64, _vp]),
     "soar_view_buffer_bytes": (C.c_int, [C.c_int32, C.c_int32, C.c_int32, C.c_int64, C.c_int32, C.POINTER(C.c_size_t)]),
     "soar_views_grad_scratch_floats": (C.c_int, [C.c_int32, C.c_int32, C.POINTER(C.c_size_t)]),
diff --git a/soar_amd/step_plan.py b/soar_amd/step_plan.py
--- a/soar_amd/step_plan.py
+++ b/soar_amd/step_plan.py
@@ -114,6 +114,9 @@
         self.optimizer_in_two_parts = None
         self.graphs = None
         self._ids_by_value = not use_graphs and self.n <= 8
+        self.fused_gather = self._ids_by_value and os.environ.get("SOAR_PLAN_FUSED_GATHER", "1") != "0"
+        self.fused_finish = os.environ.get("SOAR_PLAN_FUSED_FINISH", "1") != "0"
+        self._finish_rides = False
         if use_graphs:
             if os.environ.get("DEBUG_CLR_GRAPH_PACKET_CAPTURE") != "0":
                 raise RuntimeError("FrameStepPlan(use_graphs=True) needs DEBUG_CLR_GRAPH_PACKET_CAPTURE=0 in the environment "
@@ -234,8 +237,9 @@
         n_sets = int(self.pool.shape[0]) if self.pool is not None else 0
         if self._ids_by_value:
             ids = (C.c_int32 * self.n)(*self._frames_now)
-            check(L.soar_gather_step_inputs_ids(self.n, s.num_frames, 55 * 16, n_sets, ids, ptr(s.cano2live), ptr(self.mats),
-                                                ptr(self.frame_sel), stream), "gather_step_inputs")
+            gather = L.soar_gather_step_inputs_ids_fused if self.fused_gather else L.soar_gather_step_inputs_ids
+            check(gather(self.n, s.num_frames, 55 * 16, n_sets, ids, ptr(s.cano2live), ptr(self.mats), ptr(self.frame_sel), stream),
+                  "gather_step_inputs")
         else:
             check(L.soar_gather_step_inputs(self.n, s.num_frames, 55 * 16, n_sets, ptr(self.frame_ids), ptr(s.cano2live), ptr(self.mats),
                                             ptr(self.frame_sel), stream), "gather_step_inputs")
@@ -285,17 +289,18 @@
             L, v, W, H = self.L, self.views[i], self.W, self.H
             wc, wm, wn, wd = self.weights
             if self.pool is not None:
-                return (L.soar_frame_loss_pooled, (W, H, ptr(v["color"]), ptr(v["normal"]), ptr(v["depth"]), ptr(v["opac"]), ptr(self.pool),
+                return (L.soar_frame_loss_pooled_fused_finish if rides else L.soar_frame_loss_pooled, (W, H, ptr(v["color"]), ptr(v["normal"]), ptr(v["depth"]), ptr(v["opac"]), ptr(self.pool),
                                                    int(self.pool.shape[0]), ptr(self.frame_sel[i]), wc, wm, wn, wd, ptr(self.losses[i]),
                                                    ptr(v["sums"]), ptr(v["gC"]), ptr(v["gN"]), ptr(v["gD"]), ptr(v["gO"]), ptr(v["img"]),
                                                    self.ctx.params.bg_dev, int(self.ctx.params.cfg_normalize_depth), stream),
                         "frame_loss_pooled")
             tc, tm, tn = self.targets
-            return (L.soar_frame_loss, (W, H, ptr(v["color"]), ptr(v["normal"]), ptr(v["depth"]), ptr(v["opac"]), ptr(tc), ptr(tm), ptr(tn),
+            return (L.soar_frame_loss_fused_finish if rides else L.soar_frame_loss, (W, H, ptr(v["color"]), ptr(v["normal"]), ptr(v["depth"]), ptr(v["opac"]), ptr(tc), ptr(tm), ptr(tn),
                                         wc, wm, wn, wd, ptr(self.losses[i]), ptr(v["sums"]), ptr(v["gC"]), ptr(v["gN"]), ptr(v["gD"]),
                                         ptr(v["gO"]), ptr(v["img"]), self.ctx.params.bg_dev, int(self.ctx.params.cfg_normalize_depth), stream),
                     "frame_loss")
-        self._call(("loss", i, stream), build)
+        rides = self._finish_rides
+        self._call(("loss", i, stream, rides), build)
 
     def _f_backward(self, i: int, stream: int) -> None:
         def build():
@@ -359,7 +364,11 @@
                     v = self.views[i]
                     torch.add(torch.dot(v["terms"], self.av_coef), v["occ_terms"][0] * self.av_occ_up[0], out=self.losses[i])
         else:
-            batch((self._f_geometry, self._f_render, self._f_loss, self._f_backward))
+            self._finish_rides = self.fused_finish
+            try:
+                batch((self._f_geometry, self._f_render, self._f_loss, self._f_backward))
+            finally:
+                self._finish_rides = False
         for i in frames:
             self._stamp(3 + 2 * i, stream)
 
```

Result: no change. 5290, median of 6 (+0.6%).
